# uclanlp/visualbert

Measured on NVIDIA H100. Metric: image-text pairs/sec fwd+bwd VisualBERT-base, higher is better.
Workload: dtype bf16

## Files before the change

include/vbert_b200.h:

```cpp
#ifndef VBERT_B200_H
#define VBERT_B200_H

#include <stdint.h>

#ifdef __cplusplus
extern "C" {
#endif

#define VB_ABI_VERSION 2

int vb_abi_version(void);
const char* vb_last_error(void);
int64_t vb_launch_count(void);
#define VB_PROFILE_CATEGORIES 11
void vb_profile_enable(int on);
int vb_profile_read(double* ms, double* work, int64_t* launches);

#define VB_EPI_NONE 0
#define VB_EPI_GELU 1
#define VB_EPI_DGELU 2

typedef struct {
    const void* A; int64_t lda; int32_t a_mn_major;
    const void* B; int64_t ldb; int32_t b_mn_major;
    int32_t M, N, K;
    void* D; int64_t ldd;
    int32_t d_fp32;
    int32_t splits;
    const float* bias;
    const void* addend; int64_t ld_add;
    int32_t epilogue;
    const void* aux_in;
    void* aux_out;
    int64_t ld_aux;
    float dropout_p; uint64_t dropout_seed; uint32_t dropout_stream;
    int32_t gp_tiled;
    const void* delta_ctx; float* delta_out; int32_t delta_seq;
} vb_gemm_args;
int vb_gemm_delta_ok(int32_t M, int32_t N);
int vb_gemm_gp_tiled_ok(int32_t M, int32_t N);

int vb_gemm(const vb_gemm_args* args, void* stream);

int vb_layernorm_fwd(const void* x, int64_t ldx, const float* gamma, const float* beta, void* y, int64_t ldy,
                     float* mean, float* rstd, int32_t rows, int32_t hidden, float eps, void* stream);
int vb_layernorm_bwd(const void* dy, const void* x, const float* mean, const float* rstd, const float* gamma,
                     void* dx, void* dx_drop, float* dgamma, float* dbeta, float* dbias, int32_t rows,
                     int32_t hidden, float dropout_p, uint64_t dropout_seed, uint32_t dropout_stream,
                     float in_dropout_p, uint32_t in_dropout_stream, void* stream);

int64_t vb_attention_keep_bytes(int32_t batch, int32_t seq, int32_t heads);
int vb_attention_fwd(const void* qkv, const float* mask_bias, void* ctx, float* lse, void* keep_mask, int32_t batch,
                     int32_t seq, int32_t heads, int32_t hidden, float dropout_p, uint64_t dropout_seed,
                     uint32_t dropout_stream, void* stream);
int vb_attention_bwd(const void* qkv, const float* mask_bias, const void* ctx, const float* lse, const void* keep_mask,
                     const void* dctx, void* dqkv, float* drow, int32_t batch, int32_t seq, int32_t heads,
                     int32_t hidden, float dropout_p, uint64_t dropout_seed, uint32_t dropout_stream, void* stream);

int vb_mask_bias(const int64_t* input_mask, const int64_t* image_mask, float* out, int32_t batch, int32_t text_len,
                 int32_t num_regions, void* stream);
int vb_cast_f32_to_bf16(const float* src, void* dst, int64_t n, void* stream);
int vb_cast_bf16_to_f32(const void* src, float* dst, int64_t n, void* stream);
#define VB_CAST_CHUNK 8192
typedef struct {
    const void* src;
    void* dst;
    int64_t numel;
    int32_t first_chunk;
    int32_t dst_fp32;
} vb_cast_item;
int vb_cast_multi(const vb_cast_item* table, int32_t n_items, int32_t n_chunks, void* stream);
int vb_colsum_bf16(const void* x, int64_t ld, float* out, int32_t rows, int32_t cols, void* stream);

int vb_cross_entropy_fwd(const void* logits, int64_t ld, const int64_t* labels, int32_t rows, int32_t vocab, float* lse,
                         float* loss_rows, void* stream);
int vb_cross_entropy_bwd(void* logits, int64_t ld, const int64_t* labels, int32_t rows, int32_t vocab, int32_t padded_cols,
                         const float* lse, const float* scale, void* stream);

typedef struct {
    int32_t batch, seq, hidden, heads, inter;
    float hidden_dropout, attn_dropout;
    uint64_t seed;
    uint32_t layer_index;
    const void* w_qkv;
    const void* w_attn_out;
    const void* w_inter;
    const void* w_out;
    const float* b_qkv;
    const float* b_attn_out; const float* ln1_gamma; const float* ln1_beta;
    const float* b_inter;
    const float* b_out; const float* ln2_gamma; const float* ln2_beta;
    const float* mask_bias;
} vb_layer_desc;

typedef struct {
    void* qkv;
    void* ctx;
    float* lse;
    void* pre1;
    float* mean1; float* rstd1;
    void* x1;
    void* u;
    void* g;
    void* pre2;
    float* mean2; float* rstd2;
    void* keep_mask;
} vb_layer_acts;

typedef struct {
    float* dw_qkv; float* db_qkv; float* dw_attn_out; float* db_attn_out; float* dln1_gamma; float* dln1_beta;
    float* dw_inter; float* db_inter; float* dw_out; float* db_out; float* dln2_gamma; float* dln2_beta;
} vb_layer_grads;

typedef struct {
    void* d_pre;
    void* d_pre_drop;
    void* d_big;
    void* d_x1;
    void* d_ctx;
    float* drow;
} vb_layer_scratch;

int vb_layer_fwd(const vb_layer_desc* d, const void* x_in, void* x_out, const vb_layer_acts* acts, void* stream);
int vb_layer_bwd(const vb_layer_desc* d, const void* x_in, const vb_layer_acts* acts, const void* dy, void* dx,
                 const vb_layer_grads* grads, const vb_layer_scratch* scratch, void* stream);

#define VB_ENCODER_ARENA_BUFFERS 14
int64_t vb_encoder_arena_layout(int32_t batch, int32_t seq, int32_t hidden, int32_t heads, int32_t inter, int32_t attn_dropout_on,
                                int64_t* offsets );
int vb_encoder_fwd(const vb_layer_desc* descs, int32_t n_layers, const void* x_in, void* arena, void* stream);
int vb_encoder_bwd(const vb_layer_desc* descs, int32_t n_layers, const void* x_in, void* arena, const void* dy, void* dx,
                   const vb_layer_grads* grads, const vb_layer_scratch* scratch, void* stream);

typedef struct {
    int32_t batch, text_len, num_regions, hidden, visual_dim, vocab, max_pos, n_types;
    float eps, dropout; uint64_t seed;
    const int64_t* input_ids;
    const int64_t* token_type_ids;
    const int64_t* visual_type;
    const void* visual_feats;
    const void* w_proj;
    const float* b_proj;
    const float* word; const float* pos; const float* type; const float* pos_vis; const float* type_vis;
    const float* gamma; const float* beta;
    const void* visual_addend;
} vb_embed_desc;

typedef struct {
    void* vis_proj;
    void* pre;
    float* mean; float* rstd;
} vb_embed_acts;

typedef struct {
    float* dword; float* dpos; float* dtype; float* dpos_vis; float* dtype_vis;
    float* dw_proj; float* db_proj; float* dgamma; float* dbeta;
    void* d_pre;
    void* d_vis;
    void* d_feats;
} vb_embed_grads;

int vb_embed_fwd(const vb_embed_desc* d, void* y, const vb_embed_acts* acts, void* stream);
int vb_embed_bwd(const vb_embed_desc* d, const vb_embed_acts* acts, const void* dy, const vb_embed_grads* g, void* stream);

#define VB_ADAM_CHUNK 32768
typedef struct {
    void* p;
    const void* g;
    void* m;
    void* v;
    int64_t numel;
    float lr;
    float weight_decay;
    int32_t first_chunk;
    int32_t reserved;
} vb_adam_tensor;
int vb_bert_adam_step(const vb_adam_tensor* table, int32_t n_tensors, int32_t n_chunks, float* sumsq, double b1, double b2,
                      double eps, double max_grad_norm, void* stream);

#ifdef __cplusplus
}
#endif
#endif
```

visualbert_b200/_lib.py:

```python
import ctypes
import os

_HERE = os.path.dirname(os.path.abspath(__file__))
LIB_PATH = os.environ.get("VB_LIB_PATH") or os.path.join(_HERE, "lib", "libvbert_b200.so")

ABI_VERSION = 2
VB_EPI_NONE, VB_EPI_GELU, VB_EPI_DGELU = 0, 1, 2

c_void_p, c_int, c_i64, c_f32, c_u64, c_u32 = (
    ctypes.c_void_p, ctypes.c_int32, ctypes.c_int64, ctypes.c_float, ctypes.c_uint64, ctypes.c_uint32)


class GemmArgs(ctypes.Structure):
    _fields_ = [
        ("A", c_void_p), ("lda", c_i64), ("a_mn_major", c_int),
        ("B", c_void_p), ("ldb", c_i64), ("b_mn_major", c_int),
        ("M", c_int), ("N", c_int), ("K", c_int),
        ("D", c_void_p), ("ldd", c_i64),
        ("d_fp32", c_int), ("splits", c_int),
        ("bias", c_void_p),
        ("addend", c_void_p), ("ld_add", c_i64),
        ("epilogue", c_int),
        ("aux_in", c_void_p), ("aux_out", c_void_p), ("ld_aux", c_i64),
        ("dropout_p", c_f32), ("dropout_seed", c_u64), ("dropout_stream", c_u32),
        ("gp_tiled", c_int),
        ("delta_ctx", c_void_p), ("delta_out", c_void_p), ("delta_seq", c_int),
    ]


def _struct(name, fields):
    return type(name, (ctypes.Structure,), {"_fields_": fields})


_P = c_void_p
LayerDesc = _struct("LayerDesc", [
    ("batch", c_int), ("seq", c_int), ("hidden", c_int), ("heads", c_int), ("inter", c_int),
    ("hidden_dropout", c_f32), ("attn_dropout", c_f32), ("seed", c_u64), ("layer_index", c_u32),
    ("w_qkv", _P), ("w_attn_out", _P), ("w_inter", _P), ("w_out", _P),
    ("b_qkv", _P), ("b_attn_out", _P), ("ln1_gamma", _P), ("ln1_beta", _P),
    ("b_inter", _P), ("b_out", _P), ("ln2_gamma", _P), ("ln2_beta", _P), ("mask_bias", _P)])
LayerActs = _struct("LayerActs", [(n, _P) for n in (
    "qkv", "ctx", "lse", "pre1", "mean1", "rstd1", "x1", "u", "g", "pre2", "mean2", "rstd2", "keep_mask")])
LayerGrads = _struct("LayerGrads", [(n, _P) for n in (
    "dw_qkv", "db_qkv", "dw_attn_out", "db_attn_out", "dln1_gamma", "dln1_beta",
    "dw_inter", "db_inter", "dw_out", "db_out", "dln2_gamma", "dln2_beta")])
LayerScratch = _struct("LayerScratch", [(n, _P) for n in ("d_pre", "d_pre_drop", "d_big", "d_x1", "d_ctx", "drow")])
EmbedDesc = _struct("EmbedDesc", [
    ("batch", c_int), ("text_len", c_int), ("num_regions", c_int), ("hidden", c_int), ("visual_dim", c_int),
    ("vocab", c_int), ("max_pos", c_int), ("n_types", c_int),
    ("eps", c_f32), ("dropout", c_f32), ("seed", c_u64),
    ("input_ids", _P), ("token_type_ids", _P), ("visual_type", _P), ("visual_feats", _P),
    ("w_proj", _P), ("b_proj", _P),
    ("word", _P), ("pos", _P), ("type", _P), ("pos_vis", _P), ("type_vis", _P), ("gamma", _P), ("beta", _P),
    ("visual_addend", _P)])
EmbedActs = _struct("EmbedActs", [(n, _P) for n in ("vis_proj", "pre", "mean", "rstd")])
EmbedGrads = _struct("EmbedGrads", [(n, _P) for n in (
    "dword", "dpos", "dtype", "dpos_vis", "dtype_vis", "dw_proj", "db_proj", "dgamma", "dbeta",
    "d_pre", "d_vis", "d_feats")])

AdamTensor = _struct("AdamTensor", [
    ("p", _P), ("g", _P), ("m", _P), ("v", _P), ("numel", c_i64), ("lr", c_f32), ("weight_decay", c_f32),
    ("first_chunk", c_int), ("reserved", c_int)])
VB_ADAM_CHUNK = 32768
CastItem = _struct("CastItem", [("src", _P), ("dst", _P), ("numel", c_i64), ("first_chunk", c_int), ("dst_fp32", c_int)])
VB_CAST_CHUNK = 8192

EXPORTS = [
    "vb_abi_version", "vb_last_error", "vb_launch_count", "vb_profile_enable", "vb_profile_read", "vb_gemm", "vb_gemm_gp_tiled_ok", "vb_gemm_delta_ok", "vb_layernorm_fwd", "vb_layernorm_bwd",
    "vb_attention_keep_bytes", "vb_attention_fwd", "vb_attention_bwd", "vb_mask_bias", "vb_cast_f32_to_bf16", "vb_cast_bf16_to_f32",
    "vb_colsum_bf16", "vb_cross_entropy_fwd", "vb_cross_entropy_bwd", "vb_layer_fwd", "vb_layer_bwd", "vb_embed_fwd", "vb_embed_bwd",
    "vb_bert_adam_step", "vb_cast_multi", "vb_encoder_arena_layout", "vb_encoder_fwd", "vb_encoder_bwd",
]
VB_ENCODER_ARENA_BUFFERS = 14
ARENA_NAMES = ("qkv", "ctx", "lse", "pre1", "mean1", "rstd1", "x1", "u", "g", "pre2", "mean2", "rstd2", "keep_mask", "y")


class VBertLibraryError(RuntimeError):
    pass


_lib = None


def lib():
    global _lib
    if _lib is None:
        if not os.path.exists(LIB_PATH):
            raise VBertLibraryError(
                f"{LIB_PATH} not found: build it with `python -c 'import __graft_entry__ as g; g.build()'`. "
                "visualbert_b200 has no CPU or PyTorch fallback.")
        h = ctypes.CDLL(LIB_PATH)
        h.vb_last_error.restype = ctypes.c_char_p
        h.vb_launch_count.restype = ctypes.c_int64
        h.vb_abi_version.restype = ctypes.c_int
        h.vb_attention_keep_bytes.restype = ctypes.c_int64
        h.vb_encoder_arena_layout.restype = ctypes.c_int64
        _lib = h
    return _lib


def check(rc, what):
    if rc != 0:
        msg = lib().vb_last_error().decode("utf-8", "replace")
        raise VBertLibraryError(f"{what} failed (status {rc}): {msg}")


def launch_count():
    return int(lib().vb_launch_count())


PROFILE_CATEGORIES = ("gemm_fwd", "gemm_dgrad", "gemm_wgrad", "attn_fwd", "attn_dq", "attn_dkv", "ln_fwd", "ln_bwd",
                      "colsum", "embed", "other")


def profile_enable(on=True):
    lib().vb_profile_enable(1 if on else 0)


def profile_read():
    k = len(PROFILE_CATEGORIES)
    ms = (ctypes.c_double * k)(); work = (ctypes.c_double * k)(); n = (ctypes.c_int64 * k)()
    check(lib().vb_profile_read(ms, work, n), "vb_profile_read")
    return {c: dict(ms=ms[i], work=work[i], launches=int(n[i])) for i, c in enumerate(PROFILE_CATEGORIES)}
```

visualbert_b200/csrc/vb_api.cu:

```cuda
#include <string.h>

#include "vb_internal.h"

namespace vb {

constexpr float kLnEps = 1e-12f;
constexpr unsigned kEmbedDropStream = 0xE0000001u;
enum { kSiteAttnProbs = 0, kSiteAttnOut = 1, kSiteFfnOut = 2 };
static inline unsigned drop_stream(unsigned layer, unsigned site) { return layer * 8u + site; }

#define VB_TRY(expr)            \
    do {                        \
        int _rc = (expr);       \
        if (_rc) return _rc;    \
    } while (0)

static vb_gemm_args fwd_args(const void* A, const void* W, void* D, int M, int N, int K) {
    vb_gemm_args a;
    memset(&a, 0, sizeof(a));
    a.A = A; a.lda = K; a.B = W; a.ldb = K; a.M = M; a.N = N; a.K = K; a.D = D; a.ldd = N;
    return a;
}
static vb_gemm_args dgrad_args(const void* dY, const void* W, void* dX, int M, int N, int K) {
    vb_gemm_args a;
    memset(&a, 0, sizeof(a));
    a.A = dY; a.lda = N; a.B = W; a.ldb = K; a.b_mn_major = 1; a.M = M; a.N = K; a.K = N; a.D = dX; a.ldd = K;
    return a;
}
static vb_gemm_args wgrad_args(const void* dY, const void* X, float* dW, int M, int N, int K) {
    vb_gemm_args a;
    memset(&a, 0, sizeof(a));
    a.A = dY; a.lda = N; a.a_mn_major = 1; a.B = X; a.ldb = K; a.b_mn_major = 1;
    a.M = N; a.N = K; a.K = M; a.D = dW; a.ldd = K; a.d_fp32 = 1;
    const int tiles = ((N + 127) / 128) * ((K + 255) / 256);
    int splits = (2 * num_sms()) / tiles;
    a.splits = splits < 1 ? 1 : splits;
    return a;
}

static int check_layer(const vb_layer_desc* d) {
    VB_REQUIRE(d != nullptr, "layer: null descriptor");
    VB_REQUIRE(d->batch > 0 && d->seq > 0, "layer: empty batch");
    VB_REQUIRE(d->hidden == d->heads * 64, "layer: hidden (%d) must equal heads (%d) * 64", d->hidden, d->heads);
    VB_REQUIRE(d->hidden % 16 == 0 && d->inter % 16 == 0, "layer: hidden/intermediate must be multiples of 16");
    VB_REQUIRE(d->w_qkv && d->w_attn_out && d->w_inter && d->w_out && d->mask_bias, "layer: null weight pointer");
    return 0;
}

int layer_fwd(const vb_layer_desc* d, const void* x_in, void* x_out, const vb_layer_acts* s, cudaStream_t st) {
    VB_TRY(check_layer(d));
    VB_REQUIRE(x_in && x_out && s, "layer_fwd: null pointer");
    const int M = d->batch * d->seq, H = d->hidden, I = d->inter;
    vb_gemm_args a = fwd_args(x_in, d->w_qkv, s->qkv, M, 3 * H, H);
    a.bias = d->b_qkv;
    static cudaEvent_t before_qkv[kMaxDevices] = {nullptr};
    const int dev = current_device();
    const bool want_mask = d->attn_dropout > 0.f && s->keep_mask != nullptr;
    if (want_mask) {
        if (before_qkv[dev] == nullptr) VB_CHECK_CUDA(cudaEventCreateWithFlags(&before_qkv[dev], cudaEventDisableTiming));
        VB_CHECK_CUDA(cudaEventRecord(before_qkv[dev], st));
    }
    VB_TRY(gemm(a, st));
    int mask_ready = 0;
    if (want_mask) {
        mask_ready = attn_mask_async(s->keep_mask, d->batch, d->seq, d->heads, H, d->attn_dropout, d->seed,
                                     drop_stream(d->layer_index, kSiteAttnProbs), before_qkv[dev], st);
        if (mask_ready < 0) return 2;
    }
    VB_TRY(attn_fwd(s->qkv, d->mask_bias, s->ctx, s->lse, s->keep_mask, d->batch, d->seq, d->heads, H, d->attn_dropout, d->seed,
                    drop_stream(d->layer_index, kSiteAttnProbs), st, mask_ready == 1));
    a = fwd_args(s->ctx, d->w_attn_out, s->pre1, M, H, H);
    a.bias = d->b_attn_out; a.addend = x_in; a.ld_add = H;
    a.dropout_p = d->hidden_dropout; a.dropout_seed = d->seed; a.dropout_stream = drop_stream(d->layer_index, kSiteAttnOut);
    VB_TRY(gemm(a, st));
    VB_TRY(ln_fwd(s->pre1, H, d->ln1_gamma, d->ln1_beta, s->x1, H, s->mean1, s->rstd1, M, H, kLnEps, st));
    a = fwd_args(s->x1, d->w_inter, s->u, M, I, H);
    a.bias = d->b_inter; a.epilogue = VB_EPI_GELU; a.aux_out = s->g; a.ld_aux = I;
    a.gp_tiled = gemm_gp_tiled_ok(M, I) ? 1 : 0;
    VB_TRY(gemm(a, st));
    a = fwd_args(s->g, d->w_out, s->pre2, M, H, I);
    a.bias = d->b_out; a.addend = s->x1; a.ld_add = H;
    a.dropout_p = d->hidden_dropout; a.dropout_seed = d->seed; a.dropout_stream = drop_stream(d->layer_index, kSiteFfnOut);
    VB_TRY(gemm(a, st));
    VB_TRY(ln_fwd(s->pre2, H, d->ln2_gamma, d->ln2_beta, x_out, H, s->mean2, s->rstd2, M, H, kLnEps, st));
    return 0;
}

int layer_bwd(const vb_layer_desc* d, const void* x_in, const vb_layer_acts* s, const void* dy, void* dx,
              const vb_layer_grads* g, const vb_layer_scratch* w, cudaStream_t st) {
    VB_TRY(check_layer(d));
    VB_REQUIRE(x_in && s && dy && dx && g && w, "layer_bwd: null pointer");
    const int M = d->batch * d->seq, H = d->hidden, I = d->inter;
    const bool hd = d->hidden_dropout > 0.f;
    VB_REQUIRE(!hd || w->d_pre_drop, "layer_bwd: d_pre_drop scratch required when hidden_dropout > 0");
    void* dpm = hd ? w->d_pre_drop : w->d_pre;

    VB_TRY(ln_bwd(dy, s->pre2, s->mean2, s->rstd2, d->ln2_gamma, w->d_pre, hd ? w->d_pre_drop : nullptr, g->dln2_gamma,
                  g->dln2_beta, g->db_out, M, H, d->hidden_dropout, d->seed, drop_stream(d->layer_index, kSiteFfnOut),
                  0.f, 0, st));
    VB_TRY(gemm(wgrad_args(dpm, s->g, g->dw_out, M, H, I), st));
    vb_gemm_args a = dgrad_args(dpm, d->w_out, w->d_big, M, H, I);
    a.epilogue = VB_EPI_DGELU; a.aux_in = s->u; a.ld_aux = I;
    a.gp_tiled = gemm_gp_tiled_ok(M, I) ? 1 : 0;
    VB_TRY(gemm(a, st));
    VB_TRY(colsum(w->d_big, I, g->db_inter, M, I, st));
    VB_TRY(gemm(wgrad_args(w->d_big, s->x1, g->dw_inter, M, I, H), st));
    a = dgrad_args(w->d_big, d->w_inter, w->d_x1, M, I, H);
    a.addend = w->d_pre; a.ld_add = H;
    VB_TRY(gemm(a, st));
    VB_TRY(ln_bwd(w->d_x1, s->pre1, s->mean1, s->rstd1, d->ln1_gamma, w->d_pre, hd ? w->d_pre_drop : nullptr,
                  g->dln1_gamma, g->dln1_beta, g->db_attn_out, M, H, d->hidden_dropout, d->seed,
                  drop_stream(d->layer_index, kSiteAttnOut), 0.f, 0, st));
    VB_TRY(gemm(wgrad_args(dpm, s->ctx, g->dw_attn_out, M, H, H), st));
    a = dgrad_args(dpm, d->w_attn_out, w->d_ctx, M, H, H);
    const bool fused_delta = gemm_delta_ok(M, H) && w->drow != nullptr &&
                             attn_bwd_takes_delta(s->qkv, w->d_ctx, w->d_big, d->batch, d->seq, d->heads, H);
    if (fused_delta) { a.delta_ctx = s->ctx; a.delta_out = w->drow; a.delta_seq = d->seq; }
    VB_TRY(gemm(a, st));
    VB_TRY(attn_bwd(s->qkv, d->mask_bias, s->ctx, s->lse, s->keep_mask, w->d_ctx, w->d_big, w->drow, d->batch, d->seq, d->heads, H,
                    d->attn_dropout, d->seed, drop_stream(d->layer_index, kSiteAttnProbs), st, fused_delta));
    VB_TRY(colsum(w->d_big, 3 * H, g->db_qkv, M, 3 * H, st));
    VB_TRY(gemm(wgrad_args(w->d_big, x_in, g->dw_qkv, M, 3 * H, H), st));
    a = dgrad_args(w->d_big, d->w_qkv, dx, M, 3 * H, H);
    a.addend = w->d_pre; a.ld_add = H;
    VB_TRY(gemm(a, st));
    return 0;
}

static long long align256(long long x) { return (x + 255) / 256 * 256; }

long long encoder_arena_layout(int B, int S, int H, int A, int I, int attn_drop, long long* off) {
    const long long M = static_cast<long long>(B) * S;
    const long long sizes[VB_ENCODER_ARENA_BUFFERS] = {
        M * 3 * H * 2, M * H * 2, static_cast<long long>(B) * A * S * 4, M * H * 2, M * 4, M * 4, M * H * 2, M * I * 2, M * I * 2,
        M * H * 2, M * 4, M * 4, attn_drop ? attn_keep_bytes(B, S, A) : 0, M * H * 2};
    long long o = 0;
    for (int i = 0; i < VB_ENCODER_ARENA_BUFFERS; ++i) {
        if (off) off[i] = o;
        o += align256(sizes[i]);
    }
    return o;
}

static void arena_acts(const vb_layer_desc* d, void* arena, int l, vb_layer_acts* a, void** y) {
    long long off[VB_ENCODER_ARENA_BUFFERS];
    const long long stride = encoder_arena_layout(d->batch, d->seq, d->hidden, d->heads, d->inter, d->attn_dropout > 0.f, off);
    char* base = static_cast<char*>(arena) + l * stride;
    a->qkv = base + off[0]; a->ctx = base + off[1]; a->lse = reinterpret_cast<float*>(base + off[2]);
    a->pre1 = base + off[3]; a->mean1 = reinterpret_cast<float*>(base + off[4]); a->rstd1 = reinterpret_cast<float*>(base + off[5]);
    a->x1 = base + off[6]; a->u = base + off[7]; a->g = base + off[8]; a->pre2 = base + off[9];
    a->mean2 = reinterpret_cast<float*>(base + off[10]); a->rstd2 = reinterpret_cast<float*>(base + off[11]);
    a->keep_mask = d->attn_dropout > 0.f ? base + off[12] : nullptr;
    *y = base + off[13];
}

int encoder_fwd(const vb_layer_desc* descs, int n, const void* x_in, void* arena, cudaStream_t st) {
    VB_REQUIRE(descs && n > 0 && x_in && arena, "encoder_fwd: null pointer / no layers");
    const void* x = x_in;
    for (int l = 0; l < n; ++l) {
        VB_REQUIRE(descs[l].batch == descs[0].batch && descs[l].seq == descs[0].seq && descs[l].hidden == descs[0].hidden &&
                   descs[l].heads == descs[0].heads && descs[l].inter == descs[0].inter &&
                   (descs[l].attn_dropout > 0.f) == (descs[0].attn_dropout > 0.f), "encoder_fwd: layers differ in shape");
        vb_layer_acts a;
        void* y;
        arena_acts(&descs[l], arena, l, &a, &y);
        VB_TRY(layer_fwd(&descs[l], x, y, &a, st));
        x = y;
    }
    return 0;
}

int encoder_bwd(const vb_layer_desc* descs, int n, const void* x_in, void* arena, const void* dy, void* dx,
                const vb_layer_grads* grads, const vb_layer_scratch* w, cudaStream_t st) {
    VB_REQUIRE(descs && n > 0 && x_in && arena && dy && dx && grads && w, "encoder_bwd: null pointer / no layers");
    const void* g_in = dy;
    for (int l = n - 1; l >= 0; --l) {
        vb_layer_acts a;
        void* y;
        arena_acts(&descs[l], arena, l, &a, &y);
        const void* xl = x_in;
        if (l > 0) {
            vb_layer_acts ap;
            void* yp;
            arena_acts(&descs[l - 1], arena, l - 1, &ap, &yp);
            xl = yp;
        }
        VB_TRY(layer_bwd(&descs[l], xl, &a, g_in, dx, &grads[l], w, st));
        g_in = dx;
    }
    return 0;
}

static int check_embed(const vb_embed_desc* d) {
    VB_REQUIRE(d != nullptr, "embed: null descriptor");
    VB_REQUIRE(d->batch > 0 && d->text_len > 0 && d->num_regions >= 0, "embed: bad shape");
    VB_REQUIRE(d->hidden % 16 == 0, "embed: hidden must be a multiple of 16");
    VB_REQUIRE(d->num_regions == 0 || (d->visual_dim % 8 == 0 && d->visual_feats && d->w_proj && d->visual_type),
               "embed: visual inputs missing or visual_dim not a multiple of 8");
    return 0;
}

int embed_fwd_api(const vb_embed_desc* d, void* y, const vb_embed_acts* s, cudaStream_t st) {
    VB_TRY(check_embed(d));
    VB_REQUIRE(y && s && s->pre && s->mean && s->rstd, "embed_fwd: null pointer");
    const int BV = d->batch * d->num_regions;
    if (BV > 0) {
        vb_gemm_args a = fwd_args(d->visual_feats, d->w_proj, s->vis_proj, BV, d->hidden, d->visual_dim);
        a.bias = d->b_proj;
        if (d->visual_addend != nullptr) {
            a.addend = d->visual_addend;
            a.ld_add = d->hidden;
        }
        VB_TRY(gemm(a, st));
    }
    EmbedParams p;
    memset(&p, 0, sizeof(p));
    p.ids = reinterpret_cast<const long long*>(d->input_ids);
    p.tt = reinterpret_cast<const long long*>(d->token_type_ids);
    p.vt = reinterpret_cast<const long long*>(d->visual_type);
    p.vis_proj = static_cast<const bf16*>(s->vis_proj);
    p.word = d->word; p.pos = d->pos; p.type = d->type; p.pos_vis = d->pos_vis; p.type_vis = d->type_vis;
    p.gamma = d->gamma; p.beta = d->beta;
    p.pre = static_cast<bf16*>(s->pre); p.y = static_cast<bf16*>(y); p.mean = s->mean; p.rstd = s->rstd;
    p.B = d->batch; p.T = d->text_len; p.V = d->num_regions; p.H = d->hidden;
    p.vocab = d->vocab; p.max_pos = d->max_pos; p.n_types = d->n_types;
    p.eps = d->eps;
    if (d->dropout > 0.f) {
        const DropQ q = dropout_quantise(d->dropout);
        p.drop_scale = q.scale;
        p.drop_thresh16 = q.thr8;
        p.drop_seed = d->seed;
        p.drop_stream = kEmbedDropStream;
    }
    return embed_fwd(p, st);
}

int embed_bwd_api(const vb_embed_desc* d, const vb_embed_acts* s, const void* dy, const vb_embed_grads* g,
                  cudaStream_t st) {
    VB_TRY(check_embed(d));
    VB_REQUIRE(s && dy && g && g->d_pre, "embed_bwd: null pointer");
    const int M = d->batch * (d->text_len + d->num_regions), H = d->hidden, BV = d->batch * d->num_regions;
    VB_TRY(ln_bwd(dy, s->pre, s->mean, s->rstd, d->gamma, g->d_pre, nullptr, g->dgamma, g->dbeta, nullptr, M, H, 0.f,
                  d->seed, 0, d->dropout, kEmbedDropStream, st));
    EmbedBwdParams p;
    memset(&p, 0, sizeof(p));
    p.de = static_cast<const bf16*>(g->d_pre);
    p.ids = reinterpret_cast<const long long*>(d->input_ids);
    p.tt = reinterpret_cast<const long long*>(d->token_type_ids);
    p.vt = reinterpret_cast<const long long*>(d->visual_type);
    p.dword = g->dword; p.dpos = g->dpos; p.dtype = g->dtype; p.dpos_vis = g->dpos_vis; p.dtype_vis = g->dtype_vis;
    p.dvis = static_cast<bf16*>(g->d_vis);
    p.B = d->batch; p.T = d->text_len; p.V = d->num_regions; p.H = H;
    p.vocab = d->vocab; p.max_pos = d->max_pos; p.n_types = d->n_types;
    VB_TRY(embed_bwd(p, st));
    if (BV > 0) {
        VB_TRY(colsum(g->d_vis, H, g->db_proj, BV, H, st));
        VB_TRY(gemm(wgrad_args(g->d_vis, d->visual_feats, g->dw_proj, BV, H, d->visual_dim), st));
        if (g->d_feats) VB_TRY(gemm(dgrad_args(g->d_vis, d->w_proj, g->d_feats, BV, H, d->visual_dim), st));
    }
    return 0;
}

}

extern "C" {
int vb_layer_fwd(const vb_layer_desc* d, const void* x_in, void* x_out, const vb_layer_acts* acts, void* stream) {
    return vb::layer_fwd(d, x_in, x_out, acts, static_cast<cudaStream_t>(stream));
}
int vb_layer_bwd(const vb_layer_desc* d, const void* x_in, const vb_layer_acts* acts, const void* dy, void* dx,
                 const vb_layer_grads* grads, const vb_layer_scratch* scratch, void* stream) {
    return vb::layer_bwd(d, x_in, acts, dy, dx, grads, scratch, static_cast<cudaStream_t>(stream));
}
int64_t vb_encoder_arena_layout(int32_t batch, int32_t seq, int32_t hidden, int32_t heads, int32_t inter, int32_t attn_dropout_on,
                                int64_t* offsets) {
    long long off[VB_ENCODER_ARENA_BUFFERS];
    const long long stride = vb::encoder_arena_layout(batch, seq, hidden, heads, inter, attn_dropout_on, off);
    if (offsets) for (int i = 0; i < VB_ENCODER_ARENA_BUFFERS; ++i) offsets[i] = off[i];
    return stride;
}
int vb_encoder_fwd(const vb_layer_desc* descs, int32_t n_layers, const void* x_in, void* arena, void* stream) {
    return vb::encoder_fwd(descs, n_layers, x_in, arena, static_cast<cudaStream_t>(stream));
}
int vb_encoder_bwd(const vb_layer_desc* descs, int32_t n_layers, const void* x_in, void* arena, const void* dy, void* dx,
                   const vb_layer_grads* grads, const vb_layer_scratch* scratch, void* stream) {
    return vb::encoder_bwd(descs, n_layers, x_in, arena, dy, dx, grads, scratch, static_cast<cudaStream_t>(stream));
}
int vb_embed_fwd(const vb_embed_desc* d, void* y, const vb_embed_acts* acts, void* stream) {
    return vb::embed_fwd_api(d, y, acts, static_cast<cudaStream_t>(stream));
}
int vb_embed_bwd(const vb_embed_desc* d, const vb_embed_acts* acts, const void* dy, const vb_embed_grads* g, void* stream) {
    return vb::embed_bwd_api(d, acts, dy, g, static_cast<cudaStream_t>(stream));
}
int vb_mask_bias(const int64_t* input_mask, const int64_t* image_mask, float* out, int32_t batch, int32_t text_len,
                 int32_t num_regions, void* stream) {
    return vb::mask_bias(reinterpret_cast<const long long*>(input_mask), reinterpret_cast<const long long*>(image_mask),
                         out, batch, text_len, num_regions, static_cast<cudaStream_t>(stream));
}
int vb_cast_f32_to_bf16(const float* src, void* dst, int64_t n, void* stream) {
    return vb::cast_f32_bf16(src, dst, n, static_cast<cudaStream_t>(stream));
}
int vb_cast_bf16_to_f32(const void* src, float* dst, int64_t n, void* stream) {
    return vb::cast_bf16_f32(src, dst, n, static_cast<cudaStream_t>(stream));
}
int vb_colsum_bf16(const void* x, int64_t ld, float* out, int32_t rows, int32_t cols, void* stream) {
    return vb::colsum(x, ld, out, rows, cols, static_cast<cudaStream_t>(stream));
}
}
```

visualbert_b200/csrc/vb_common.cuh:

```cuda
#pragma once

#include <cuda.h>
#include <cuda_bf16.h>
#include <cuda_runtime.h>
#include <stdint.h>
#include <stdio.h>

#include <atomic>

namespace vb {

typedef __nv_bfloat16 bf16;

extern std::atomic<long long> g_launches;
int num_sms();
constexpr int kMaxDevices = 64;
int current_device();
template <typename K>
inline cudaError_t ensure_dyn_smem(K kern, int bytes, int (&cache)[kMaxDevices]) {
    const int d = current_device();
    if (cache[d] >= bytes) return cudaSuccess;
    cudaError_t e = cudaFuncSetAttribute(kern, cudaFuncAttributeMaxDynamicSharedMemorySize, bytes);
    if (e == cudaSuccess) cache[d] = bytes;
    return e;
}

enum { PROF_GEMM_FWD = 0, PROF_GEMM_DGRAD = 1, PROF_GEMM_WGRAD = 2, PROF_ATTN_FWD = 3, PROF_ATTN_DQ = 4, PROF_ATTN_DKV = 5,
       PROF_LN_FWD = 6, PROF_LN_BWD = 7, PROF_COLSUM = 8, PROF_EMBED = 9, PROF_OTHER = 10, PROF_NCAT = 11 };
bool pdl_enabled();
#ifdef __CUDACC__
__device__ __forceinline__ void pdl_wait() { asm volatile("griddepcontrol.wait;" ::: "memory"); }
__device__ __forceinline__ void pdl_trigger() { asm volatile("griddepcontrol.launch_dependents;" ::: "memory"); }
template <typename... KArgs, typename... Args>
inline cudaError_t launch_pdl(void (*kernel)(KArgs...), dim3 grid, dim3 block, size_t smem, cudaStream_t st, Args&&... args) {
    cudaLaunchConfig_t cfg = {};
    cfg.gridDim = grid;
    cfg.blockDim = block;
    cfg.dynamicSmemBytes = smem;
    cfg.stream = st;
    cudaLaunchAttribute attr[1];
    attr[0].id = cudaLaunchAttributeProgrammaticStreamSerialization;
    attr[0].val.programmaticStreamSerializationAllowed = 1;
    cfg.attrs = attr;
    cfg.numAttrs = pdl_enabled() ? 1 : 0;
    return cudaLaunchKernelEx(&cfg, kernel, static_cast<KArgs>(args)...);
}
#endif

struct ProfScope {
    ProfScope(cudaStream_t st, int cat, double work, int launches);
    ~ProfScope();
    int slot;
    cudaStream_t st;
};

void set_error(const char* fmt, ...);
#define VB_CHECK_CUDA(expr)                                                                   \
    do {                                                                                      \
        cudaError_t _e = (expr);                                                              \
        if (_e != cudaSuccess) {                                                              \
            vb::set_error("%s:%d: %s -> %s", __FILE__, __LINE__, #expr, cudaGetErrorString(_e)); \
            return 1;                                                                         \
        }                                                                                     \
    } while (0)
#define VB_REQUIRE(cond, ...)                                                                 \
    do {                                                                                      \
        if (!(cond)) {                                                                        \
            vb::set_error(__VA_ARGS__);                                                       \
            return 2;                                                                         \
        }                                                                                     \
    } while (0)

__device__ __forceinline__ uint32_t smem_u32(const void* p) {
    return static_cast<uint32_t>(__cvta_generic_to_shared(p));
}

__device__ __forceinline__ float warp_sum(float v) {
#pragma unroll
    for (int o = 16; o > 0; o >>= 1) v += __shfl_xor_sync(0xffffffffu, v, o);
    return v;
}
__device__ __forceinline__ float warp_max(float v) {
#pragma unroll
    for (int o = 16; o > 0; o >>= 1) v = fmaxf(v, __shfl_xor_sync(0xffffffffu, v, o));
    return v;
}

__device__ __forceinline__ uint32_t pack_bf16x2(float lo, float hi) {
    __nv_bfloat162 h = __floats2bfloat162_rn(lo, hi);
    return *reinterpret_cast<uint32_t*>(&h);
}
__device__ __forceinline__ float2 unpack_bf16x2(uint32_t v) {
    __nv_bfloat162 h = *reinterpret_cast<__nv_bfloat162*>(&v);
    return __bfloat1622float2(h);
}

__device__ __forceinline__ float fast_ex2(float x) {
    float r;
    asm("ex2.approx.ftz.f32 %0, %1;" : "=f"(r) : "f"(x));
    return r;
}
__device__ __forceinline__ float fast_rcp(float x) {
    float r;
    asm("rcp.approx.ftz.f32 %0, %1;" : "=f"(r) : "f"(x));
    return r;
}

__device__ __forceinline__ float erfc_abs_sqrt2(float x, float& e) {
    const float ax = fabsf(x);
    e = fast_ex2(x * x * -0.72134752044448170f);
    const float t = fast_rcp(fmaf(0.23164189f, ax, 1.0f));
    float poly = fmaf(1.061405429f, t, -1.453152027f);
    poly = fmaf(poly, t, 1.421413741f);
    poly = fmaf(poly, t, -0.284496736f);
    poly = fmaf(poly, t, 0.254829592f);
    return poly * t * e;
}
__device__ __forceinline__ float gelu_fwd(float x) {
    float e;
    const float q = erfc_abs_sqrt2(x, e);
    const float hx = 0.5f * x, ha = fabsf(hx);
    return fmaf(-ha, q, hx + ha);
}
__device__ __forceinline__ void gelu_fwd_bwd(float x, float& g, float& gp) {
    float e;
    const float q = erfc_abs_sqrt2(x, e);
    const float cdf = 0.5f + copysignf(fmaf(-0.5f, q, 0.5f), x);
    g = x * cdf;
    gp = fmaf(x * e, 0.3989422804014327f, cdf);
}
__device__ __forceinline__ float gelu_bwd(float x) {
    float e;
    const float q = erfc_abs_sqrt2(x, e);
    const float cdf = 0.5f + copysignf(fmaf(-0.5f, q, 0.5f), x);
    return fmaf(x * e, 0.3989422804014327f, cdf);
}

__device__ __forceinline__ uint32_t mix32(uint32_t x) {
    x ^= x >> 16; x *= 0x7feb352du;
    x ^= x >> 15; x *= 0x846ca68bu;
    x ^= x >> 16;
    return x;
}
__device__ __forceinline__ uint32_t dropout_key(uint64_t seed, uint32_t stream) {
    return mix32(static_cast<uint32_t>(seed) ^ mix32(static_cast<uint32_t>(seed >> 32) + 0x9E3779B9u * (stream + 1u)));
}
struct DropQ { unsigned thr8; float scale; };
inline DropQ dropout_quantise(float p) {
    DropQ q;
    unsigned n = static_cast<unsigned>(p * 256.0f + 0.5f);
    if (n > 255u) n = 255u;
    q.thr8 = n;
    q.scale = p > 0.f ? 256.0f / (256.0f - static_cast<float>(n)) : 0.f;
    return q;
}
__device__ __forceinline__ uint32_t dropout_keep8(uint64_t seed, uint32_t stream, uint64_t elem8, uint32_t thr8) {
    const uint32_t key = dropout_key(seed, stream) ^ (static_cast<uint32_t>(elem8 >> 31) * 0x27d4eb2fu);
    const uint32_t base = static_cast<uint32_t>(elem8) << 1;
    const uint32_t t4 = thr8 * 0x01010101u;
    const uint32_t m0 = __vcmpgeu4(mix32(base ^ key), t4) & 0x01010101u;
    const uint32_t m1 = __vcmpgeu4(mix32((base + 1u) ^ key), t4) & 0x01010101u;
    return ((m0 * 0x01020408u) >> 24) | (((m1 * 0x01020408u) >> 24) << 4);
}

__device__ __forceinline__ void mbar_init(uint32_t bar, uint32_t count) {
    asm volatile("mbarrier.init.shared::cta.b64 [%0], %1;" ::"r"(bar), "r"(count) : "memory");
}
__device__ __forceinline__ void fence_barrier_init() {
    asm volatile("fence.mbarrier_init.release.cluster;" ::: "memory");
}
__device__ __forceinline__ void fence_proxy_async_smem() {
    asm volatile("fence.proxy.async.shared::cta;" ::: "memory");
}
__device__ __forceinline__ void mbar_arrive(uint32_t bar) {
    asm volatile("mbarrier.arrive.shared::cta.b64 _, [%0];" ::"r"(bar) : "memory");
}
__device__ __forceinline__ void mbar_arrive_expect_tx(uint32_t bar, uint32_t bytes) {
    asm volatile("mbarrier.arrive.expect_tx.shared::cta.b64 _, [%0], %1;" ::"r"(bar), "r"(bytes)
                 : "memory");
}
__device__ __forceinline__ bool mbar_try_wait(uint32_t bar, uint32_t parity) {
    uint32_t ok;
    asm volatile(
        "{\n"
        ".reg .pred p;\n"
        "mbarrier.try_wait.parity.shared::cta.b64 p, [%1], %2;\n"
        "selp.u32 %0, 1, 0, p;\n"
        "}\n"
        : "=r"(ok)
        : "r"(bar), "r"(parity)
        : "memory");
    return ok != 0;
}
__device__ __forceinline__ void mbar_wait(uint32_t bar, uint32_t parity) {
    if (mbar_try_wait(bar, parity)) return;
    const long long t0 = clock64();
    uint32_t spins = 0;
    while (!mbar_try_wait(bar, parity)) {
        if ((++spins & 0x3ffu) == 0 && clock64() - t0 > 4000000000ll) __trap();
    }
}

__device__ __forceinline__ void tma_prefetch_desc(const CUtensorMap* m) {
    asm volatile("prefetch.tensormap [%0];" ::"l"(reinterpret_cast<uint64_t>(m)) : "memory");
}
__device__ __forceinline__ void tma_load_2d(uint32_t smem_dst, const CUtensorMap* m, uint32_t bar,
                                            int c_inner, int c_outer) {
    asm volatile(
        "cp.async.bulk.tensor.2d.shared::cluster.global.mbarrier::complete_tx::bytes"
        " [%0], [%1, {%3, %4}], [%2];"
        ::"r"(smem_dst), "l"(reinterpret_cast<uint64_t>(m)), "r"(bar), "r"(c_inner), "r"(c_outer)
        : "memory");
}

__device__ __forceinline__ uint64_t wgmma_desc_sw128(uint32_t saddr, uint32_t lbo_bytes, uint32_t sbo_bytes) {
    return static_cast<uint64_t>((saddr & 0x3FFFFu) >> 4) | (static_cast<uint64_t>((lbo_bytes >> 4) & 0x3FFFu) << 16) |
           (static_cast<uint64_t>((sbo_bytes >> 4) & 0x3FFFu) << 32) | (1ull << 62);
}
__device__ __forceinline__ void wgmma_fence() { asm volatile("wgmma.fence.sync.aligned;" ::: "memory"); }
__device__ __forceinline__ void wgmma_commit() { asm volatile("wgmma.commit_group.sync.aligned;" ::: "memory"); }
template <int N>
__device__ __forceinline__ void wgmma_wait() { asm volatile("wgmma.wait_group.sync.aligned %0;" ::"n"(N) : "memory"); }
template <int TA, int TB>
__device__ __forceinline__ void wgmma_m64n128k16(float (&d)[64], uint64_t a_desc, uint64_t b_desc, uint32_t accumulate) {
    asm volatile(
        "{\n"
        ".reg .pred p;\n"
        "setp.ne.b32 p, %66, 0;\n"
        "wgmma.mma_async.sync.aligned.m64n128k16.f32.bf16.bf16 "
        "{%0, %1, %2, %3, %4, %5, %6, %7, %8, %9, %10, %11, %12, %13, %14, %15, %16, %17, %18, %19, %20, %21, %22, %23, %24, %25, %26, %27, %28, %29, %30, %31, %32, %33, %34, %35, %36, %37, %38, %39, %40, %41, %42, %43, %44, %45, %46, %47, %48, %49, %50, %51, %52, %53, %54, %55, %56, %57, %58, %59, %60, %61, %62, %63}, "
        "%64, %65, p, 1, 1, %67, %68;\n"
        "}\n"
        : "+f"(d[0]), "+f"(d[1]), "+f"(d[2]), "+f"(d[3]), "+f"(d[4]), "+f"(d[5]), "+f"(d[6]), "+f"(d[7]),
          "+f"(d[8]), "+f"(d[9]), "+f"(d[10]), "+f"(d[11]), "+f"(d[12]), "+f"(d[13]), "+f"(d[14]), "+f"(d[15]),
          "+f"(d[16]), "+f"(d[17]), "+f"(d[18]), "+f"(d[19]), "+f"(d[20]), "+f"(d[21]), "+f"(d[22]), "+f"(d[23]),
          "+f"(d[24]), "+f"(d[25]), "+f"(d[26]), "+f"(d[27]), "+f"(d[28]), "+f"(d[29]), "+f"(d[30]), "+f"(d[31]),
          "+f"(d[32]), "+f"(d[33]), "+f"(d[34]), "+f"(d[35]), "+f"(d[36]), "+f"(d[37]), "+f"(d[38]), "+f"(d[39]),
          "+f"(d[40]), "+f"(d[41]), "+f"(d[42]), "+f"(d[43]), "+f"(d[44]), "+f"(d[45]), "+f"(d[46]), "+f"(d[47]),
          "+f"(d[48]), "+f"(d[49]), "+f"(d[50]), "+f"(d[51]), "+f"(d[52]), "+f"(d[53]), "+f"(d[54]), "+f"(d[55]),
          "+f"(d[56]), "+f"(d[57]), "+f"(d[58]), "+f"(d[59]), "+f"(d[60]), "+f"(d[61]), "+f"(d[62]), "+f"(d[63])
        : "l"(a_desc), "l"(b_desc), "r"(accumulate), "n"(TA), "n"(TB));
}
template <int TA, int TB>
__device__ __forceinline__ void wgmma_m64n64k16_ss(float (&d)[32], uint64_t a_desc, uint64_t b_desc, uint32_t accumulate) {
    asm volatile(
        "{\n"
        ".reg .pred p;\n"
        "setp.ne.b32 p, %34, 0;\n"
        "wgmma.mma_async.sync.aligned.m64n64k16.f32.bf16.bf16 "
        "{%0, %1, %2, %3, %4, %5, %6, %7, %8, %9, %10, %11, %12, %13, %14, %15, %16, %17, %18, %19, %20, %21, %22, %23, %24, %25, %26, %27, %28, %29, %30, %31}, "
        "%32, %33, p, 1, 1, %35, %36;\n"
        "}\n"
        : "+f"(d[0]), "+f"(d[1]), "+f"(d[2]), "+f"(d[3]), "+f"(d[4]), "+f"(d[5]), "+f"(d[6]), "+f"(d[7]),
          "+f"(d[8]), "+f"(d[9]), "+f"(d[10]), "+f"(d[11]), "+f"(d[12]), "+f"(d[13]), "+f"(d[14]), "+f"(d[15]),
          "+f"(d[16]), "+f"(d[17]), "+f"(d[18]), "+f"(d[19]), "+f"(d[20]), "+f"(d[21]), "+f"(d[22]), "+f"(d[23]),
          "+f"(d[24]), "+f"(d[25]), "+f"(d[26]), "+f"(d[27]), "+f"(d[28]), "+f"(d[29]), "+f"(d[30]), "+f"(d[31])
        : "l"(a_desc), "l"(b_desc), "r"(accumulate), "n"(TA), "n"(TB));
}
template <int TB>
__device__ __forceinline__ void wgmma_m64n64k16_rs(float (&d)[32], const uint32_t (&a)[4], uint64_t b_desc, uint32_t accumulate) {
    asm volatile(
        "{\n"
        ".reg .pred p;\n"
        "setp.ne.b32 p, %37, 0;\n"
        "wgmma.mma_async.sync.aligned.m64n64k16.f32.bf16.bf16 "
        "{%0, %1, %2, %3, %4, %5, %6, %7, %8, %9, %10, %11, %12, %13, %14, %15, %16, %17, %18, %19, %20, %21, %22, %23, %24, %25, %26, %27, %28, %29, %30, %31}, "
        "{%32, %33, %34, %35}, %36, p, 1, 1, %38;\n"
        "}\n"
        : "+f"(d[0]), "+f"(d[1]), "+f"(d[2]), "+f"(d[3]), "+f"(d[4]), "+f"(d[5]), "+f"(d[6]), "+f"(d[7]),
          "+f"(d[8]), "+f"(d[9]), "+f"(d[10]), "+f"(d[11]), "+f"(d[12]), "+f"(d[13]), "+f"(d[14]), "+f"(d[15]),
          "+f"(d[16]), "+f"(d[17]), "+f"(d[18]), "+f"(d[19]), "+f"(d[20]), "+f"(d[21]), "+f"(d[22]), "+f"(d[23]),
          "+f"(d[24]), "+f"(d[25]), "+f"(d[26]), "+f"(d[27]), "+f"(d[28]), "+f"(d[29]), "+f"(d[30]), "+f"(d[31])
        : "r"(a[0]), "r"(a[1]), "r"(a[2]), "r"(a[3]), "l"(b_desc), "r"(accumulate), "n"(TB));
}
__device__ __forceinline__ bool elect_one() {
    uint32_t pred;
    asm volatile(
        "{\n"
        ".reg .pred P1;\n"
        "elect.sync _|P1, 0xffffffff;\n"
        "selp.u32 %0, 1, 0, P1;\n"
        "}\n"
        : "=r"(pred));
    return pred != 0;
}
template <int N>
__device__ __forceinline__ void reg_dec() { asm volatile("setmaxnreg.dec.sync.aligned.u32 %0;" ::"n"(N)); }
template <int N>
__device__ __forceinline__ void reg_inc() { asm volatile("setmaxnreg.inc.sync.aligned.u32 %0;" ::"n"(N)); }
__device__ __forceinline__ void named_bar_sync(int id, int nthreads) {
    asm volatile("bar.sync %0, %1;" ::"r"(id), "r"(nthreads) : "memory");
}

__device__ __forceinline__ uint4 ldg_v4(const void* p) {
    return __ldg(reinterpret_cast<const uint4*>(p));
}
__device__ __forceinline__ void stg_v4(void* p, uint4 v) { *reinterpret_cast<uint4*>(p) = v; }
__device__ __forceinline__ void ldg_v8(const void* p, uint32_t (&r)[8]) {
    const uint4 a = ldg_v4(p), b = ldg_v4(static_cast<const uint8_t*>(p) + 16);
    r[0] = a.x; r[1] = a.y; r[2] = a.z; r[3] = a.w; r[4] = b.x; r[5] = b.y; r[6] = b.z; r[7] = b.w;
}
__device__ __forceinline__ void stg_v8(void* p, const uint32_t (&r)[8]) {
    stg_v4(p, make_uint4(r[0], r[1], r[2], r[3]));
    stg_v4(static_cast<uint8_t*>(p) + 16, make_uint4(r[4], r[5], r[6], r[7]));
}
__device__ __forceinline__ void red_add_v4_f32(float* p, float a, float b, float c, float d) {
    asm volatile("red.global.add.v4.f32 [%0], {%1, %2, %3, %4};" ::"l"(p), "f"(a), "f"(b), "f"(c),
                 "f"(d)
                 : "memory");
}

}
```

visualbert_b200/csrc/vb_gemm.cu:

```cuda
#include <stdarg.h>
#include <stdio.h>
#include <stdlib.h>
#include <string.h>

#include <atomic>
#include <mutex>
#include <vector>

#include "../../include/vbert_b200.h"
#include "vb_common.cuh"

namespace vb {

static thread_local char g_err[1024] = "";
std::atomic<long long> g_launches{0};

void set_error(const char* fmt, ...) {
    va_list ap;
    va_start(ap, fmt);
    vsnprintf(g_err, sizeof(g_err), fmt, ap);
    va_end(ap);
}
const char* get_error() { return g_err; }

struct ProfRec { cudaEvent_t e0, e1; int cat; double work; int launches; };
static bool g_prof_on = false;
static std::vector<ProfRec> g_prof;
static std::vector<ProfRec> g_prof_pool;
static std::mutex g_prof_mu;

ProfScope::ProfScope(cudaStream_t s, int cat, double work, int launches) : slot(-1), st(s) {
    g_launches.fetch_add(launches);
    if (!g_prof_on) return;
    std::lock_guard<std::mutex> lk(g_prof_mu);
    ProfRec r;
    if (!g_prof_pool.empty()) { r = g_prof_pool.back(); g_prof_pool.pop_back(); }
    else { cudaEventCreate(&r.e0); cudaEventCreate(&r.e1); }
    r.cat = cat; r.work = work; r.launches = launches;
    cudaEventRecord(r.e0, st);
    g_prof.push_back(r);
    slot = static_cast<int>(g_prof.size()) - 1;
}
ProfScope::~ProfScope() {
    if (slot < 0) return;
    std::lock_guard<std::mutex> lk(g_prof_mu);
    cudaEventRecord(g_prof[slot].e1, st);
}

constexpr int BLOCK_M = 128;
constexpr int BLOCK_K = 64;
constexpr int WGMMA_K = 16;
constexpr int kStages = 4;
constexpr int kEpiWarps = 8;
constexpr int kThreads = 128 + kEpiWarps * 32;
constexpr int kAtomBytes = 64 * BLOCK_K * 2;

template <int BLOCK_N>
struct Cfg {
    static constexpr int A_BYTES = BLOCK_M * BLOCK_K * 2;
    static constexpr int B_BYTES = BLOCK_N * BLOCK_K * 2;
    static constexpr int STAGE_BYTES = A_BYTES + B_BYTES;
    static constexpr int ACC_LD = BLOCK_N + 4;
    static constexpr int RING_BYTES = kStages * STAGE_BYTES > BLOCK_M * ACC_LD * 4 ? kStages * STAGE_BYTES : BLOCK_M * ACC_LD * 4;
    static constexpr int BAR_OFF = RING_BYTES;
    static constexpr int NUM_BARS = 2 * kStages;
    static constexpr int BIAS_OFF = BAR_OFF + NUM_BARS * 8;
    static constexpr int SMEM_BYTES = BIAS_OFF + BLOCK_N * 4 + 1024;
    static_assert(SMEM_BYTES <= 227 * 1024, "shared memory per block");
};

struct GemmParams {
    int M, N, K;
    int splits;
    void* D; long long ldd;
    const float* bias;
    const bf16* addend; long long ld_add;
    int epilogue;
    const bf16* aux_in;
    bf16* aux_out; long long ld_aux;
    float drop_scale;
    unsigned drop_thresh16;
    unsigned long long drop_seed;
    unsigned drop_stream;
    int m_fast;
    float* delta_out;
    int delta_seq;
};
bool gemm_gp_tiled_ok(int M, int N);
bool gemm_delta_ok(int M, int N);

struct TileCoord {
    int m_blk, n_blk, kb_begin, kb_end;
};
__device__ __forceinline__ TileCoord decode_tile(int t, int n_blocks, int splits, int k_blocks, int m_blocks, bool m_fast) {
    TileCoord c;
    const int split = t % splits;
    const int mn = t / splits;
    if (m_fast) {
        c.m_blk = mn % m_blocks;
        c.n_blk = mn / m_blocks;
    } else {
        c.n_blk = mn % n_blocks;
        c.m_blk = mn / n_blocks;
    }
    c.kb_begin = static_cast<int>(static_cast<long long>(split) * k_blocks / splits);
    c.kb_end = static_cast<int>(static_cast<long long>(split + 1) * k_blocks / splits);
    return c;
}

__device__ __forceinline__ void load16_bf16(const bf16* p, float (&f)[16]) {
    uint32_t r[8];
    ldg_v8(p, r);
#pragma unroll
    for (int i = 0; i < 8; ++i) {
        const float2 t = unpack_bf16x2(r[i]);
        f[2 * i] = t.x;
        f[2 * i + 1] = t.y;
    }
}
__device__ __forceinline__ void store16_bf16(bf16* p, const float (&f)[16]) {
    uint32_t r[8];
#pragma unroll
    for (int i = 0; i < 8; ++i) r[i] = pack_bf16x2(f[2 * i], f[2 * i + 1]);
    stg_v8(p, r);
}

enum { EPI_GENERIC = 0, EPI_BIAS = 1, EPI_RESID = 2, EPI_DROP_RESID = 3, EPI_GELU_FWD = 4, EPI_DGELU_BWD = 5, EPI_GELU_FWD_T = 6,
       EPI_DGELU_BWD_T = 7, EPI_DELTA = 8 };
__host__ __device__ constexpr bool epi_is_gelu(int e) { return e == EPI_GELU_FWD || e == EPI_GELU_FWD_T; }
__host__ __device__ constexpr bool epi_is_dgelu(int e) { return e == EPI_DGELU_BWD || e == EPI_DGELU_BWD_T; }

template <bool OUT_F32, int EPI = EPI_GENERIC, bool TO_REGS = false>
__device__ __forceinline__ void epilogue16(const GemmParams& p, int row, int col, const float* sbias, const uint32_t (&ex)[8],
                                           float (&x)[16], uint32_t* o0 = nullptr, uint32_t* o1 = nullptr) {
    if (sbias != nullptr) {
#pragma unroll
        for (int i = 0; i < 4; ++i) {
            const float4 b = *reinterpret_cast<const float4*>(sbias + 4 * i);
            x[4 * i] += b.x; x[4 * i + 1] += b.y; x[4 * i + 2] += b.z; x[4 * i + 3] += b.w;
        }
    }
    if constexpr (OUT_F32) {
        float* d = reinterpret_cast<float*>(p.D) + static_cast<long long>(row) * p.ldd + col;
#pragma unroll
        for (int i = 0; i < 4; ++i) red_add_v4_f32(d + 4 * i, x[4 * i], x[4 * i + 1], x[4 * i + 2], x[4 * i + 3]);
    } else {
        constexpr bool kGeneric = EPI == EPI_GENERIC;
        if (EPI == EPI_DROP_RESID || (kGeneric && p.drop_scale != 0.0f)) {
            const unsigned long long e8 =
                (static_cast<unsigned long long>(row) * static_cast<unsigned>(p.N) + col) >> 3;
#pragma unroll
            for (int h = 0; h < 2; ++h) {
                const uint32_t keep = dropout_keep8(p.drop_seed, p.drop_stream, e8 + h, p.drop_thresh16);
#pragma unroll
                for (int i = 0; i < 8; ++i) x[8 * h + i] = ((keep >> i) & 1u) ? x[8 * h + i] * p.drop_scale : 0.0f;
            }
        }
        if (EPI == EPI_RESID || EPI == EPI_DROP_RESID || (kGeneric && p.addend != nullptr)) {
#pragma unroll
            for (int i = 0; i < 8; ++i) {
                const float2 t = unpack_bf16x2(ex[i]);
                x[2 * i] += t.x;
                x[2 * i + 1] += t.y;
            }
        }
        bf16* d = reinterpret_cast<bf16*>(p.D) + static_cast<long long>(row) * p.ldd + col;
        if (epi_is_gelu(EPI) || (kGeneric && p.epilogue == VB_EPI_GELU)) {
            float gp[16];
#pragma unroll
            for (int i = 0; i < 16; ++i) gelu_fwd_bwd(x[i], x[i], gp[i]);
            if constexpr (TO_REGS) {
#pragma unroll
                for (int i = 0; i < 8; ++i) { o0[i] = pack_bf16x2(gp[2 * i], gp[2 * i + 1]); o1[i] = pack_bf16x2(x[2 * i], x[2 * i + 1]); }
                return;
            }
            store16_bf16(d, gp);
            d = p.aux_out + static_cast<long long>(row) * p.ld_aux + col;
        } else if (kGeneric && p.epilogue == 3) {
            store16_bf16(d, x);
            d = p.aux_out + static_cast<long long>(row) * p.ld_aux + col;
        } else if (epi_is_dgelu(EPI) || (kGeneric && p.epilogue == VB_EPI_DGELU)) {
#pragma unroll
            for (int i = 0; i < 8; ++i) {
                const float2 t = unpack_bf16x2(ex[i]);
                x[2 * i] *= t.x;
                x[2 * i + 1] *= t.y;
            }
        }
        if constexpr (TO_REGS) {
#pragma unroll
            for (int i = 0; i < 8; ++i) o0[i] = pack_bf16x2(x[2 * i], x[2 * i + 1]);
            return;
        }
        store16_bf16(d, x);
    }
}

template <bool A_MN, bool B_MN, int BLOCK_N, bool OUT_F32, int EPI = EPI_GENERIC>
__global__ void __launch_bounds__(kThreads, 1)
gemm_wgmma_kernel(const __grid_constant__ CUtensorMap tmA, const __grid_constant__ CUtensorMap tmB, const GemmParams p) {
    using C = Cfg<BLOCK_N>;
    static_assert(BLOCK_N % 128 == 0, "64 x 128 wgmma pieces");
    static_assert(!(EPI == EPI_GELU_FWD_T || EPI == EPI_DGELU_BWD_T) || BLOCK_N == 256, "tile-native gelu' is defined on 256-wide tiles");
    extern __shared__ uint8_t smem_raw[];
    const uint32_t raw = smem_u32(smem_raw);
    const uint32_t base = (raw + 1023u) & ~1023u;
    uint8_t* smem = smem_raw + (base - raw);

    const int warp = threadIdx.x >> 5;
    const int lane = threadIdx.x & 31;

    auto a_tile = [&](int s) { return base + s * C::STAGE_BYTES; };
    auto b_tile = [&](int s) { return base + s * C::STAGE_BYTES + C::A_BYTES; };
    auto full_bar = [&](int s) { return base + C::BAR_OFF + 8 * s; };
    auto empty_bar = [&](int s) { return base + C::BAR_OFF + 8 * (kStages + s); };

    if (threadIdx.x == 0) {
        tma_prefetch_desc(&tmA);
        tma_prefetch_desc(&tmB);
        for (int s = 0; s < kStages; ++s) {
            mbar_init(full_bar(s), 1);
            mbar_init(empty_bar(s), 2);
        }
        fence_barrier_init();
    }
    __syncthreads();
    pdl_trigger();
    pdl_wait();

    const int m_blocks = (p.M + BLOCK_M - 1) / BLOCK_M;
    const int n_blocks = (p.N + BLOCK_N - 1) / BLOCK_N;
    const int k_blocks = (p.K + BLOCK_K - 1) / BLOCK_K;
    const TileCoord tc = decode_tile(blockIdx.x, n_blocks, p.splits, k_blocks, m_blocks, p.m_fast != 0);

    if (warp < 4) {
        reg_dec<40>();
        if (warp == 0) {
            int stage = 0;
            uint32_t phase = 0;
            for (int kb = tc.kb_begin; kb < tc.kb_end; ++kb) {
                mbar_wait(empty_bar(stage), phase ^ 1u);
                if (elect_one()) {
                    mbar_arrive_expect_tx(full_bar(stage), C::STAGE_BYTES);
                    if constexpr (!A_MN) {
                        tma_load_2d(a_tile(stage), &tmA, full_bar(stage), kb * BLOCK_K, tc.m_blk * BLOCK_M);
                    } else {
#pragma unroll
                        for (int i = 0; i < BLOCK_M / 64; ++i)
                            tma_load_2d(a_tile(stage) + i * kAtomBytes, &tmA, full_bar(stage), tc.m_blk * BLOCK_M + i * 64, kb * BLOCK_K);
                    }
                    if constexpr (!B_MN) {
                        tma_load_2d(b_tile(stage), &tmB, full_bar(stage), kb * BLOCK_K, tc.n_blk * BLOCK_N);
                    } else {
#pragma unroll
                        for (int i = 0; i < BLOCK_N / 64; ++i)
                            tma_load_2d(b_tile(stage) + i * kAtomBytes, &tmB, full_bar(stage), tc.n_blk * BLOCK_N + i * 64, kb * BLOCK_K);
                    }
                }
                __syncwarp();
                if (++stage == kStages) { stage = 0; phase ^= 1u; }
            }
        }
        return;
    }
    reg_inc<232>();

    const int wg = (warp >> 2) - 1;
    const int et = threadIdx.x - 128;
    float* sbias = reinterpret_cast<float*>(smem + C::BIAS_OFF);
    const bool has_bias = p.bias != nullptr;
    if (has_bias) {
        const bool mine = p.splits == 1 || (blockIdx.x % p.splits) == 0;
        for (int i = et; i < BLOCK_N; i += kEpiWarps * 32) {
            const int col = tc.n_blk * BLOCK_N + i;
            sbias[i] = (mine && col < p.N) ? __ldg(p.bias + col) : 0.f;
        }
    }
    constexpr int NH = BLOCK_N / 128;
    constexpr uint32_t a_kstep = A_MN ? WGMMA_K * 128 : WGMMA_K * 2;
    constexpr uint32_t b_kstep = B_MN ? WGMMA_K * 128 : WGMMA_K * 2;
    float acc[NH][64];
    {
        int stage = 0, prev = 0;
        uint32_t phase = 0;
        for (int kb = tc.kb_begin; kb < tc.kb_end; ++kb) {
            mbar_wait(full_bar(stage), phase);
            const uint32_t a0 = a_tile(stage) + wg * 8192, b0 = b_tile(stage);
            wgmma_fence();
#pragma unroll
            for (int k = 0; k < BLOCK_K / WGMMA_K; ++k) {
                const uint64_t ad = wgmma_desc_sw128(a0 + k * a_kstep, kAtomBytes, 1024);
#pragma unroll
                for (int h = 0; h < NH; ++h)
                    wgmma_m64n128k16<A_MN ? 1 : 0, B_MN ? 1 : 0>(acc[h], ad, wgmma_desc_sw128(b0 + h * 16384 + k * b_kstep, kAtomBytes, 1024),
                                                                 (kb > tc.kb_begin || k > 0) ? 1u : 0u);
            }
            wgmma_commit();
            wgmma_wait<1>();
            if (kb > tc.kb_begin && (threadIdx.x & 127) == 0) mbar_arrive(empty_bar(prev));
            prev = stage;
            if (++stage == kStages) { stage = 0; phase ^= 1u; }
        }
        wgmma_wait<0>();
    }

    const int ew = warp - 4;
    const int q = ew & 3, half = ew >> 2;
    const int lrow = q * 32 + lane;
    const int row = tc.m_blk * BLOCK_M + lrow;
    const int col0 = tc.n_blk * BLOCK_N + half * (BLOCK_N / 2);
    constexpr int NCH = BLOCK_N / 2 / 16;
    const long long gp_tile_off =
        ((((static_cast<long long>(tc.m_blk >> 1) * n_blocks + tc.n_blk) * 2 + (tc.m_blk & 1)) * kEpiWarps + ew) * NCH) * 512 + lane * 16;
    const bf16* exb = nullptr;
    long long ex_step = 16;
    if constexpr (!OUT_F32) {
        constexpr bool kWantAdd = EPI == EPI_RESID || EPI == EPI_DROP_RESID || EPI == EPI_DELTA;
        if (row < p.M) {
            if (kWantAdd || (EPI == EPI_GENERIC && p.addend != nullptr)) exb = p.addend + static_cast<long long>(row) * p.ld_add + col0;
            else if (EPI == EPI_DGELU_BWD || (EPI == EPI_GENERIC && p.epilogue == VB_EPI_DGELU))
                exb = p.aux_in + static_cast<long long>(row) * p.ld_aux + col0;
            else if (EPI == EPI_DGELU_BWD_T) { exb = p.aux_in + gp_tile_off; ex_step = 512; }
        }
    }
    constexpr bool kEx = !OUT_F32 && EPI != EPI_BIAS && !epi_is_gelu(EPI);
    uint32_t ex[kEx ? NCH : 1][8];
    if constexpr (kEx) {
#pragma unroll
        for (int k = 0; k < NCH; ++k)
            if (exb != nullptr && col0 + k * 16 < p.N) ldg_v8(exb + k * ex_step, ex[k]);
    }

    named_bar_sync(1, kEpiWarps * 32);
    float* sacc = reinterpret_cast<float*>(smem);
    {
        const int r0 = wg * 64 + ((warp & 3) << 4) + (lane >> 2);
#pragma unroll
        for (int h = 0; h < NH; ++h)
#pragma unroll
            for (int j = 0; j < 16; ++j)
#pragma unroll
                for (int i = 0; i < 2; ++i)
                    *reinterpret_cast<float2*>(sacc + (r0 + 8 * i) * C::ACC_LD + h * 128 + j * 8 + 2 * (lane & 3)) =
                        make_float2(acc[h][4 * j + 2 * i], acc[h][4 * j + 2 * i + 1]);
    }
    named_bar_sync(1, kEpiWarps * 32);

    const float* srow = sacc + lrow * C::ACC_LD + half * (BLOCK_N / 2);
    [[maybe_unused]] float hsum = 0.f;
#pragma unroll
    for (int k = 0; k < NCH; ++k) {
        const int col = col0 + k * 16;
        if (row < p.M && col < p.N) {
            float x[16];
#pragma unroll
            for (int i = 0; i < 4; ++i) {
                const float4 v = *reinterpret_cast<const float4*>(srow + k * 16 + 4 * i);
                x[4 * i] = v.x; x[4 * i + 1] = v.y; x[4 * i + 2] = v.z; x[4 * i + 3] = v.w;
            }
            const float* sb = has_bias ? sbias + half * (BLOCK_N / 2) + k * 16 : nullptr;
            const uint32_t (&e)[8] = ex[kEx ? k : 0];
            if constexpr (EPI == EPI_GELU_FWD_T) {
                uint32_t o0[8], o1[8];
                epilogue16<OUT_F32, EPI, true>(p, row, col, sb, e, x, o0, o1);
                stg_v8(reinterpret_cast<bf16*>(p.D) + gp_tile_off + k * 512, o0);
                stg_v8(p.aux_out + static_cast<long long>(row) * p.ld_aux + col, o1);
            } else if constexpr (EPI == EPI_DELTA) {
                uint32_t o0[8];
                epilogue16<OUT_F32, EPI, true>(p, row, col, sb, e, x, o0);
                stg_v8(reinterpret_cast<bf16*>(p.D) + static_cast<long long>(row) * p.ldd + col, o0);
#pragma unroll
                for (int i = 0; i < 8; ++i) {
                    const float2 a = unpack_bf16x2(o0[i]), b = unpack_bf16x2(e[i]);
                    hsum = fmaf(a.x, b.x, fmaf(a.y, b.y, hsum));
                }
            } else {
                epilogue16<OUT_F32, EPI>(p, row, col, sb, e, x);
            }
        }
        if constexpr (EPI == EPI_DELTA) {
            if ((k & 3) == 3) {
                const int c4 = col - 48;
                if (row < p.M && c4 < p.N) {
                    const int bi = row / p.delta_seq, si = row - bi * p.delta_seq;
                    p.delta_out[(static_cast<long long>(bi) * (p.N >> 6) + (c4 >> 6)) * p.delta_seq + si] = hsum;
                }
                hsum = 0.f;
            }
        }
    }
}

typedef CUresult (*EncodeTiledFn)(CUtensorMap*, CUtensorMapDataType, cuuint32_t, void*, const cuuint64_t*,
                                  const cuuint64_t*, const cuuint32_t*, const cuuint32_t*,
                                  CUtensorMapInterleave, CUtensorMapSwizzle, CUtensorMapL2promotion,
                                  CUtensorMapFloatOOBfill);

static EncodeTiledFn get_encode_fn() {
    static EncodeTiledFn fn = nullptr;
    static bool tried = false;
    if (!tried) {
        tried = true;
        void* sym = nullptr;
        cudaDriverEntryPointQueryResult qres;
        if (cudaGetDriverEntryPoint("cuTensorMapEncodeTiled", &sym, cudaEnableDefault, &qres) == cudaSuccess &&
            qres == cudaDriverEntryPointSuccess)
            fn = reinterpret_cast<EncodeTiledFn>(sym);
    }
    return fn;
}

struct TmapKey {
    const void* ptr; uint64_t d0, d1, d2, s0, s1; uint32_t b0, b1, b2, rank; int dev;
    bool operator==(const TmapKey& o) const {
        return ptr == o.ptr && d0 == o.d0 && d1 == o.d1 && d2 == o.d2 && s0 == o.s0 && s1 == o.s1 && b0 == o.b0 && b1 == o.b1 && b2 == o.b2 &&
               rank == o.rank && dev == o.dev;
    }
};
struct TmapSlot { TmapKey key; CUtensorMap map; bool used; };
constexpr int kTmapSlots = 4096;
static thread_local std::vector<TmapSlot>* g_tmap_cache = nullptr;

static int encode_tmap_cached(CUtensorMap* m, const void* ptr, uint32_t rank, const cuuint64_t* dims, const cuuint64_t* strides,
                              const cuuint32_t* box) {
    TmapKey k;
    memset(&k, 0, sizeof(k));
    k.ptr = ptr; k.rank = rank; k.dev = current_device();
    k.d0 = dims[0]; k.d1 = dims[1]; k.d2 = rank > 2 ? dims[2] : 1;
    k.s0 = strides[0]; k.s1 = rank > 2 ? strides[1] : 0;
    k.b0 = box[0]; k.b1 = box[1]; k.b2 = rank > 2 ? box[2] : 1;
    uint64_t h = reinterpret_cast<uintptr_t>(ptr) * 0x9E3779B97F4A7C15ull;
    h ^= (k.d0 * 31 + k.d1) * 0xBF58476D1CE4E5B9ull + k.d2 * 1315423911ull + k.s0 * 2654435761ull + k.s1 * 40503ull;
    h ^= (static_cast<uint64_t>(k.b1) << 20) ^ (static_cast<uint64_t>(k.b0) << 8) ^ k.b2 ^ (static_cast<uint64_t>(k.dev) << 40);
    h ^= h >> 29;
    if (g_tmap_cache == nullptr) { g_tmap_cache = new std::vector<TmapSlot>(kTmapSlots); for (auto& sl : *g_tmap_cache) sl.used = false; }
    TmapSlot& sl = (*g_tmap_cache)[h & (kTmapSlots - 1)];
    if (sl.used && sl.key == k) { *m = sl.map; return 0; }
    EncodeTiledFn fn = get_encode_fn();
    VB_REQUIRE(fn != nullptr, "cuTensorMapEncodeTiled unavailable (driver too old / no GPU?)");
    cuuint32_t estr[3] = {1, 1, 1};
    CUresult r = fn(m, CU_TENSOR_MAP_DATA_TYPE_BFLOAT16, rank, const_cast<void*>(ptr), dims, strides, box, estr,
                    CU_TENSOR_MAP_INTERLEAVE_NONE, CU_TENSOR_MAP_SWIZZLE_128B, CU_TENSOR_MAP_L2_PROMOTION_L2_256B,
                    CU_TENSOR_MAP_FLOAT_OOB_FILL_NONE);
    VB_REQUIRE(r == CUDA_SUCCESS, "cuTensorMapEncodeTiled (rank %u) failed with CUresult %d", rank, static_cast<int>(r));
    sl.key = k; sl.map = *m; sl.used = true;
    return 0;
}

int make_tmap_bf16(CUtensorMap* m, const void* ptr, uint64_t inner, uint64_t outer, uint64_t ld_elems,
                   uint32_t box_outer) {
    VB_REQUIRE((reinterpret_cast<uintptr_t>(ptr) & 15) == 0, "TMA operand not 16-byte aligned");
    VB_REQUIRE((ld_elems * 2) % 16 == 0, "TMA operand row stride must be a multiple of 8 elements");
    cuuint64_t dims[2] = {inner, outer};
    cuuint64_t strides[1] = {ld_elems * 2};
    cuuint32_t box[2] = {64, box_outer};
    return encode_tmap_cached(m, ptr, 2, dims, strides, box);
}

int current_device() {
    int dev = 0;
    cudaGetDevice(&dev);
    return (dev < 0 || dev >= kMaxDevices) ? 0 : dev;
}

int num_sms() {
    static int n[kMaxDevices] = {0};
    const int dev = current_device();
    if (n[dev] == 0) {
        int v = 0;
        cudaDeviceGetAttribute(&v, cudaDevAttrMultiProcessorCount, dev);
        n[dev] = v > 0 ? v : 132;
    }
    return n[dev];
}

template <bool A_MN, bool B_MN, int BLOCK_N, bool OUT_F32, int EPI = EPI_GENERIC>
static int launch(const CUtensorMap& ta, const CUtensorMap& tb, const GemmParams& p, cudaStream_t st) {
    using C = Cfg<BLOCK_N>;
    auto kern = gemm_wgmma_kernel<A_MN, B_MN, BLOCK_N, OUT_F32, EPI>;
    static int configured[kMaxDevices] = {0};
    VB_CHECK_CUDA(ensure_dyn_smem(kern, C::SMEM_BYTES, configured));
    const long long tiles = static_cast<long long>((p.M + BLOCK_M - 1) / BLOCK_M) * ((p.N + BLOCK_N - 1) / BLOCK_N) * p.splits;
    VB_REQUIRE(tiles < (1LL << 31), "vb_gemm: too many tiles");
    {
        ProfScope ps(st, OUT_F32 ? PROF_GEMM_WGRAD : (B_MN ? PROF_GEMM_DGRAD : PROF_GEMM_FWD), 2.0 * p.M * p.N * p.K, 1);
        VB_CHECK_CUDA(launch_pdl(kern, dim3(static_cast<unsigned>(tiles)), dim3(kThreads), C::SMEM_BYTES, st, ta, tb, p));
    }
    VB_CHECK_CUDA(cudaGetLastError());
    return 0;
}

bool pdl_enabled() {
    static const bool on = [] {
        const char* e = getenv("VB_PDL");
        return !(e && e[0] == '0');
    }();
    return on;
}

bool gemm_delta_ok(int M, int N) {
    static const int off = [] { const char* e = getenv("VB_GEMM_DELTA"); return (e != nullptr && atoi(e) == 0) ? 1 : 0; }();
    const int n_pad256 = (N + 255) / 256 * 256;
    return !off && M >= 256 && N >= 256 && N % 64 == 0 && (n_pad256 - N) * 8 <= N;
}
bool gemm_gp_tiled_ok(int M, int N) {
    static const int off = [] { const char* e = getenv("VB_GEMM_GP_TILED"); return (e != nullptr && atoi(e) == 0) ? 1 : 0; }();
    return !off && M >= 256 && M % 256 == 0 && N % 256 == 0;
}

int gemm(const vb_gemm_args& a, cudaStream_t st) {
    VB_REQUIRE(a.M > 0 && a.N > 0 && a.K > 0, "vb_gemm: empty problem M=%d N=%d K=%d", a.M, a.N, a.K);
    VB_REQUIRE(a.N % 16 == 0, "vb_gemm: N=%d must be a multiple of 16", a.N);
    VB_REQUIRE(a.A && a.B && a.D, "vb_gemm: null operand");
    VB_REQUIRE(a.ldd % 16 == 0 && (reinterpret_cast<uintptr_t>(a.D) & 31) == 0, "vb_gemm: D must be 32-byte aligned with ldd a multiple of 16");
    VB_REQUIRE(!a.addend || (a.ld_add % 16 == 0 && (reinterpret_cast<uintptr_t>(a.addend) & 31) == 0), "vb_gemm: addend must be 32-byte aligned with ld a multiple of 16");
    VB_REQUIRE((!a.aux_in && !a.aux_out) || a.ld_aux % 16 == 0, "vb_gemm: ld_aux must be a multiple of 16");
    VB_REQUIRE((reinterpret_cast<uintptr_t>(a.aux_in) & 31) == 0 && (reinterpret_cast<uintptr_t>(a.aux_out) & 31) == 0,
               "vb_gemm: aux_in / aux_out must be 32-byte aligned");
    VB_REQUIRE(a.epilogue == VB_EPI_NONE || a.epilogue == VB_EPI_GELU || a.epilogue == VB_EPI_DGELU || a.epilogue == 3,
               "vb_gemm: unknown epilogue %d", a.epilogue);
    VB_REQUIRE(a.epilogue != VB_EPI_GELU || a.aux_out, "vb_gemm: GELU epilogue needs aux_out");
    VB_REQUIRE(a.epilogue != VB_EPI_DGELU || a.aux_in, "vb_gemm: DGELU epilogue needs aux_in");
    VB_REQUIRE(!a.d_fp32 || (a.epilogue == VB_EPI_NONE && !a.addend && a.dropout_p == 0.0f),
               "vb_gemm: fp32-accumulate output supports bias only");
    VB_REQUIRE(a.dropout_p >= 0.0f && a.dropout_p < 1.0f, "vb_gemm: dropout_p out of range");
    VB_REQUIRE(!a.delta_out || (gemm_delta_ok(a.M, a.N) && a.delta_ctx && a.delta_seq > 0 && a.M % a.delta_seq == 0 && !a.d_fp32 &&
                                !a.a_mn_major && a.b_mn_major && !a.bias && !a.addend && a.dropout_p == 0.0f && a.epilogue == VB_EPI_NONE &&
                                (reinterpret_cast<uintptr_t>(a.delta_ctx) & 31) == 0),
               "vb_gemm: delta_out needs a plain bf16 input-gradient GEMM (b_mn_major, no bias / addend / dropout) and vb_gemm_delta_ok(M, N)");
    VB_REQUIRE(!a.gp_tiled || (gemm_gp_tiled_ok(a.M, a.N) && !a.d_fp32 && !a.a_mn_major && (a.epilogue == VB_EPI_GELU || a.epilogue == VB_EPI_DGELU)),
               "vb_gemm: gp_tiled needs a GELU / DGELU epilogue and vb_gemm_gp_tiled_ok(M, N)");
    VB_REQUIRE(!a.gp_tiled || a.epilogue != VB_EPI_DGELU || a.b_mn_major,
               "vb_gemm: gp_tiled with the DGELU epilogue needs an MN-major B (the input-gradient GEMM)");
    VB_REQUIRE(!a.gp_tiled || a.epilogue != VB_EPI_GELU || !a.b_mn_major, "vb_gemm: gp_tiled with the GELU epilogue needs a K-major B");

    GemmParams p;
    memset(&p, 0, sizeof(p));
    p.M = a.M; p.N = a.N; p.K = a.K;
    const int k_blocks = (a.K + BLOCK_K - 1) / BLOCK_K;
    int splits = (a.d_fp32 && a.splits > 1) ? a.splits : 1;
    if (splits > k_blocks) splits = k_blocks;
    p.splits = splits;
    p.D = a.D; p.ldd = a.ldd;
    p.bias = a.bias;
    p.addend = static_cast<const bf16*>(a.addend); p.ld_add = a.ld_add;
    p.epilogue = a.epilogue;
    p.aux_in = static_cast<const bf16*>(a.aux_in);
    p.aux_out = static_cast<bf16*>(a.aux_out);
    p.ld_aux = a.ld_aux;
    if (a.delta_out) {
        p.addend = static_cast<const bf16*>(a.delta_ctx); p.ld_add = a.N;
        p.delta_out = a.delta_out; p.delta_seq = a.delta_seq;
    }
    {
        static const int order_off = [] { const char* e = getenv("VB_GEMM_TILE_ORDER"); return (e != nullptr && atoi(e) == 0) ? 1 : 0; }();
        p.m_fast = (!order_off && (a.M + BLOCK_M - 1) / BLOCK_M < (a.N + 255) / 256) ? 1 : 0;
    }
    if (a.dropout_p > 0.0f) {
        const DropQ q = dropout_quantise(a.dropout_p);
        p.drop_scale = q.scale;
        p.drop_thresh16 = q.thr8;
        p.drop_seed = a.dropout_seed;
        p.drop_stream = a.dropout_stream;
    }

    const int n_pad256 = (a.N + 255) / 256 * 256;
    const bool bn256 = (a.N >= 256) && ((n_pad256 - a.N) * 8 <= a.N);
    VB_REQUIRE(!a.delta_out || bn256, "vb_gemm: delta_out needs 256-wide tiles");

    CUtensorMap ta, tb;
    int rc;
    if (!a.a_mn_major) rc = make_tmap_bf16(&ta, a.A, a.K, a.M, a.lda, BLOCK_M);
    else               rc = make_tmap_bf16(&ta, a.A, a.M, a.K, a.lda, BLOCK_K);
    if (rc) return rc;
    if (!a.b_mn_major) rc = make_tmap_bf16(&tb, a.B, a.K, a.N, a.ldb, bn256 ? 256 : 128);
    else               rc = make_tmap_bf16(&tb, a.B, a.N, a.K, a.ldb, BLOCK_K);
    if (rc) return rc;

    if (bn256 && !a.d_fp32) {
        const bool drop = a.dropout_p > 0.0f, add = a.addend != nullptr;
        int epi = EPI_GENERIC;
        if (a.epilogue == VB_EPI_GELU && !drop && !add) epi = a.gp_tiled ? EPI_GELU_FWD_T : EPI_GELU_FWD;
        else if (a.epilogue == VB_EPI_DGELU && !drop && !add) epi = a.gp_tiled ? EPI_DGELU_BWD_T : EPI_DGELU_BWD;
        else if (a.epilogue == VB_EPI_NONE) epi = add ? (drop ? EPI_DROP_RESID : EPI_RESID) : (drop ? EPI_GENERIC : EPI_BIAS);
        if (a.delta_out) epi = EPI_DELTA;
        VB_REQUIRE(!a.gp_tiled || epi == EPI_GELU_FWD_T || epi == EPI_DGELU_BWD_T,
                   "vb_gemm: gp_tiled needs a plain GELU / DGELU epilogue (no dropout, no addend)");
        if (!a.a_mn_major && !a.b_mn_major) {
            switch (epi) {
                case EPI_BIAS: return launch<false, false, 256, false, EPI_BIAS>(ta, tb, p, st);
                case EPI_RESID: return launch<false, false, 256, false, EPI_RESID>(ta, tb, p, st);
                case EPI_DROP_RESID: return launch<false, false, 256, false, EPI_DROP_RESID>(ta, tb, p, st);
                case EPI_GELU_FWD: return launch<false, false, 256, false, EPI_GELU_FWD>(ta, tb, p, st);
                case EPI_GELU_FWD_T: return launch<false, false, 256, false, EPI_GELU_FWD_T>(ta, tb, p, st);
                default: return launch<false, false, 256, false>(ta, tb, p, st);
            }
        }
        if (!a.a_mn_major && a.b_mn_major) {
            switch (epi) {
                case EPI_BIAS: return launch<false, true, 256, false, EPI_BIAS>(ta, tb, p, st);
                case EPI_RESID: return launch<false, true, 256, false, EPI_RESID>(ta, tb, p, st);
                case EPI_DGELU_BWD: return launch<false, true, 256, false, EPI_DGELU_BWD>(ta, tb, p, st);
                case EPI_DELTA: return launch<false, true, 256, false, EPI_DELTA>(ta, tb, p, st);
                case EPI_DGELU_BWD_T: return launch<false, true, 256, false, EPI_DGELU_BWD_T>(ta, tb, p, st);
                default: return launch<false, true, 256, false>(ta, tb, p, st);
            }
        }
    }

#define VB_DISPATCH(AM, BM, F32)                                         \
    (bn256 ? launch<AM, BM, 256, F32>(ta, tb, p, st) : launch<AM, BM, 128, F32>(ta, tb, p, st))
    if (!a.d_fp32) {
        if (!a.a_mn_major && !a.b_mn_major) return VB_DISPATCH(false, false, false);
        if (!a.a_mn_major && a.b_mn_major) return VB_DISPATCH(false, true, false);
        if (a.a_mn_major && a.b_mn_major) return VB_DISPATCH(true, true, false);
        return VB_DISPATCH(true, false, false);
    } else {
        if (!a.a_mn_major && !a.b_mn_major) return VB_DISPATCH(false, false, true);
        if (!a.a_mn_major && a.b_mn_major) return VB_DISPATCH(false, true, true);
        if (a.a_mn_major && a.b_mn_major) return VB_DISPATCH(true, true, true);
        return VB_DISPATCH(true, false, true);
    }
#undef VB_DISPATCH
}

}

extern "C" {
int vb_abi_version(void) { return VB_ABI_VERSION; }
const char* vb_last_error(void) { return vb::get_error(); }
int64_t vb_launch_count(void) { return vb::g_launches.load(); }
void vb_profile_enable(int on) {
    std::lock_guard<std::mutex> lk(vb::g_prof_mu);
    vb::g_prof_on = on != 0;
}
int vb_profile_read(double* ms, double* work, int64_t* launches) {
    if (cudaDeviceSynchronize() != cudaSuccess) { vb::set_error("vb_profile_read: device sync failed"); return 1; }
    std::lock_guard<std::mutex> lk(vb::g_prof_mu);
    for (int c = 0; c < vb::PROF_NCAT; ++c) { ms[c] = 0; work[c] = 0; launches[c] = 0; }
    for (auto& r : vb::g_prof) {
        float t = 0.f;
        cudaEventElapsedTime(&t, r.e0, r.e1);
        ms[r.cat] += t; work[r.cat] += r.work; launches[r.cat] += r.launches;
        vb::g_prof_pool.push_back(r);
    }
    vb::g_prof.clear();
    return 0;
}
int vb_gemm_delta_ok(int32_t M, int32_t N) { return vb::gemm_delta_ok(M, N) ? 1 : 0; }
int vb_gemm_gp_tiled_ok(int32_t M, int32_t N) { return vb::gemm_gp_tiled_ok(M, N) ? 1 : 0; }
int vb_gemm(const vb_gemm_args* args, void* stream) {
    if (!args) { vb::set_error("vb_gemm: null args"); return 2; }
    return vb::gemm(*args, static_cast<cudaStream_t>(stream));
}
}
```

visualbert_b200/csrc/vb_internal.h:

```cpp
#pragma once
#include "../../include/vbert_b200.h"
#include "vb_common.cuh"

namespace vb {

int gemm(const vb_gemm_args& a, cudaStream_t st);
bool gemm_gp_tiled_ok(int M, int N);
bool gemm_delta_ok(int M, int N);
int ln_fwd(const void* x, long long ldx, const float* gamma, const float* beta, void* y, long long ldy, float* mean,
           float* rstd, int rows, int H, float eps, cudaStream_t st);
int ln_bwd(const void* dy, const void* x, const float* mean, const float* rstd, const float* gamma, void* dx,
           void* dx_drop, float* dgamma, float* dbeta, float* dbias, int rows, int H, float dropout_p,
           unsigned long long seed, unsigned stream_id, float in_dropout_p, unsigned in_stream_id, cudaStream_t st);
int attn_fwd(const void* qkv, const float* mask_bias, void* ctx, float* lse, void* keep, int B, int S, int A, int H,
             float dropout_p, unsigned long long seed, unsigned stream_id, cudaStream_t st, bool mask_ready = false);
int attn_mask_async(void* keep, int B, int S, int A, int H, float dropout_p, unsigned long long seed, unsigned stream_id,
                    cudaEvent_t before_gemm, cudaStream_t main);
int attn_bwd(const void* qkv, const float* mask_bias, const void* ctx, const float* lse, const void* keep,
             const void* dctx, void* dqkv, float* drow, int B, int S, int A, int H, float dropout_p,
             unsigned long long seed, unsigned stream_id, cudaStream_t st, bool delta_ready = false);
bool attn_bwd_takes_delta(const void* qkv, const void* dctx, void* dqkv, int B, int S, int A, int H);
long long attn_keep_bytes(int B, int S, int A);
int colsum(const void* x, long long ld, float* out, int M, int N, cudaStream_t st);
int cast_f32_bf16(const float* src, void* dst, long long n, cudaStream_t st);
int cast_bf16_f32(const void* src, float* dst, long long n, cudaStream_t st);
int mask_bias(const long long* input_mask, const long long* image_mask, float* out, int B, int T, int V, cudaStream_t st);

struct EmbedParams {
    const long long* ids; const long long* tt; const long long* vt;
    const bf16* vis_proj;
    const float* word; const float* pos; const float* type; const float* pos_vis; const float* type_vis;
    const float* gamma; const float* beta;
    bf16* pre; bf16* y; float* mean; float* rstd;
    int B, T, V, H, vocab, max_pos, n_types;
    float eps;
    float drop_scale; unsigned drop_thresh16; unsigned long long drop_seed; unsigned drop_stream;
};
struct EmbedBwdParams {
    const bf16* de;
    const long long* ids; const long long* tt; const long long* vt;
    float* dword; float* dpos; float* dtype; float* dpos_vis; float* dtype_vis;
    bf16* dvis;
    int B, T, V, H, vocab, max_pos, n_types;
};
int embed_fwd(const EmbedParams& p, cudaStream_t st);
int embed_bwd(const EmbedBwdParams& p, cudaStream_t st);


}
```

Before: 3991.

## Make bf16 GEMM persistent with ping-pong consumer warpgroups and separate wgrad kernel

Replaces the one-tile-per-CTA bf16 GEMM with a persistent kernel whose two consumer warpgroups alternate tiles via named barriers. One warpgroup's epilogue runs while the other issues WGMMA on the next tile, and each tile is fixed at 128x128. Weight-gradient (fp32 output) GEMMs move to a separate kernel that keeps the 128/256 tile choice and uses a new split-K heuristic targeting good SM wave fill. The change adds a lot of scheduling complexity, and the tile-native GELU offset math assumes pairs of 128 tiles, which carries correctness and tuning risk.

```diff
diff --git a/include/vbert_b200.h b/include/vbert_b200.h
--- a/include/vbert_b200.h
+++ b/include/vbert_b200.h
@@ -38,6 +38,7 @@
     const void* delta_ctx; float* delta_out; int32_t delta_seq;
 } vb_gemm_args;
 int vb_gemm_delta_ok(int32_t M, int32_t N);
+int vb_gemm_wgrad_splits(int32_t M, int32_t N, int32_t K);
 int vb_gemm_gp_tiled_ok(int32_t M, int32_t N);
 
 int vb_gemm(const vb_gemm_args* args, void* stream);
diff --git a/visualbert_b200/_lib.py b/visualbert_b200/_lib.py
--- a/visualbert_b200/_lib.py
+++ b/visualbert_b200/_lib.py
@@ -66,7 +66,7 @@
 VB_CAST_CHUNK = 8192
 
 EXPORTS = [
-    "vb_abi_version", "vb_last_error", "vb_launch_count", "vb_profile_enable", "vb_profile_read", "vb_gemm", "vb_gemm_gp_tiled_ok", "vb_gemm_delta_ok", "vb_layernorm_fwd", "vb_layernorm_bwd",
+    "vb_abi_version", "vb_last_error", "vb_launch_count", "vb_profile_enable", "vb_profile_read", "vb_gemm", "vb_gemm_gp_tiled_ok", "vb_gemm_delta_ok", "vb_gemm_wgrad_splits", "vb_layernorm_fwd", "vb_layernorm_bwd",
     "vb_attention_keep_bytes", "vb_attention_fwd", "vb_attention_bwd", "vb_mask_bias", "vb_cast_f32_to_bf16", "vb_cast_bf16_to_f32",
     "vb_colsum_bf16", "vb_cross_entropy_fwd", "vb_cross_entropy_bwd", "vb_layer_fwd", "vb_layer_bwd", "vb_embed_fwd", "vb_embed_bwd",
     "vb_bert_adam_step", "vb_cast_multi", "vb_encoder_arena_layout", "vb_encoder_fwd", "vb_encoder_bwd",
diff --git a/visualbert_b200/csrc/vb_api.cu b/visualbert_b200/csrc/vb_api.cu
--- a/visualbert_b200/csrc/vb_api.cu
+++ b/visualbert_b200/csrc/vb_api.cu
@@ -32,9 +32,7 @@
     memset(&a, 0, sizeof(a));
     a.A = dY; a.lda = N; a.a_mn_major = 1; a.B = X; a.ldb = K; a.b_mn_major = 1;
     a.M = N; a.N = K; a.K = M; a.D = dW; a.ldd = K; a.d_fp32 = 1;
-    const int tiles = ((N + 127) / 128) * ((K + 255) / 256);
-    int splits = (2 * num_sms()) / tiles;
-    a.splits = splits < 1 ? 1 : splits;
+    a.splits = gemm_wgrad_splits(N, K, M);
     return a;
 }
 
diff --git a/visualbert_b200/csrc/vb_common.cuh b/visualbert_b200/csrc/vb_common.cuh
--- a/visualbert_b200/csrc/vb_common.cuh
+++ b/visualbert_b200/csrc/vb_common.cuh
@@ -192,12 +192,17 @@
         : "memory");
     return ok != 0;
 }
+__device__ __forceinline__ uint64_t global_ns() {
+    uint64_t t;
+    asm volatile("mov.u64 %0, %%globaltimer;" : "=l"(t));
+    return t;
+}
 __device__ __forceinline__ void mbar_wait(uint32_t bar, uint32_t parity) {
     if (mbar_try_wait(bar, parity)) return;
-    const long long t0 = clock64();
+    const uint64_t t0 = global_ns();
     uint32_t spins = 0;
     while (!mbar_try_wait(bar, parity)) {
-        if ((++spins & 0x3ffu) == 0 && clock64() - t0 > 4000000000ll) __trap();
+        if ((++spins & 0x3ffu) == 0 && global_ns() - t0 > 10000000000ull) __trap();
     }
 }
 
@@ -291,6 +296,9 @@
 __device__ __forceinline__ void named_bar_sync(int id, int nthreads) {
     asm volatile("bar.sync %0, %1;" ::"r"(id), "r"(nthreads) : "memory");
 }
+__device__ __forceinline__ void named_bar_arrive(int id, int nthreads) {
+    asm volatile("bar.arrive %0, %1;" ::"r"(id), "r"(nthreads) : "memory");
+}
 
 __device__ __forceinline__ uint4 ldg_v4(const void* p) {
     return __ldg(reinterpret_cast<const uint4*>(p));
diff --git a/visualbert_b200/csrc/vb_gemm.cu b/visualbert_b200/csrc/vb_gemm.cu
--- a/visualbert_b200/csrc/vb_gemm.cu
+++ b/visualbert_b200/csrc/vb_gemm.cu
@@ -48,26 +48,22 @@
 }
 
 constexpr int BLOCK_M = 128;
+constexpr int BLOCK_N = 128;
 constexpr int BLOCK_K = 64;
 constexpr int WGMMA_K = 16;
 constexpr int kStages = 4;
-constexpr int kEpiWarps = 8;
-constexpr int kThreads = 128 + kEpiWarps * 32;
+constexpr int kThreads = 384;
 constexpr int kAtomBytes = 64 * BLOCK_K * 2;
-
-template <int BLOCK_N>
-struct Cfg {
-    static constexpr int A_BYTES = BLOCK_M * BLOCK_K * 2;
-    static constexpr int B_BYTES = BLOCK_N * BLOCK_K * 2;
-    static constexpr int STAGE_BYTES = A_BYTES + B_BYTES;
-    static constexpr int ACC_LD = BLOCK_N + 4;
-    static constexpr int RING_BYTES = kStages * STAGE_BYTES > BLOCK_M * ACC_LD * 4 ? kStages * STAGE_BYTES : BLOCK_M * ACC_LD * 4;
-    static constexpr int BAR_OFF = RING_BYTES;
-    static constexpr int NUM_BARS = 2 * kStages;
-    static constexpr int BIAS_OFF = BAR_OFF + NUM_BARS * 8;
-    static constexpr int SMEM_BYTES = BIAS_OFF + BLOCK_N * 4 + 1024;
-    static_assert(SMEM_BYTES <= 227 * 1024, "shared memory per block");
-};
+constexpr int kABytes = BLOCK_M * BLOCK_K * 2;
+constexpr int kStageBytes = kABytes + BLOCK_N * BLOCK_K * 2;
+constexpr int kStgLd = BLOCK_N / 2 + 4;
+constexpr int kStgBytes = BLOCK_M * kStgLd * 4;
+constexpr int kStgOff = kStages * kStageBytes;
+constexpr int kBiasOff = kStgOff + 2 * kStgBytes;
+constexpr int kBarOff = kBiasOff + 2 * BLOCK_N * 4;
+constexpr int kSmemBytes = kBarOff + 2 * kStages * 8 + 1024;
+static_assert(kSmemBytes <= 227 * 1024, "shared memory per block");
+constexpr int kBarMmaTurn = 1, kBarEpi = 3;
 
 struct GemmParams {
     int M, N, K;
@@ -196,12 +192,9 @@
     }
 }
 
-template <bool A_MN, bool B_MN, int BLOCK_N, bool OUT_F32, int EPI = EPI_GENERIC>
+template <bool A_MN, bool B_MN, int EPI = EPI_GENERIC>
 __global__ void __launch_bounds__(kThreads, 1)
 gemm_wgmma_kernel(const __grid_constant__ CUtensorMap tmA, const __grid_constant__ CUtensorMap tmB, const GemmParams p) {
-    using C = Cfg<BLOCK_N>;
-    static_assert(BLOCK_N % 128 == 0, "64 x 128 wgmma pieces");
-    static_assert(!(EPI == EPI_GELU_FWD_T || EPI == EPI_DGELU_BWD_T) || BLOCK_N == 256, "tile-native gelu' is defined on 256-wide tiles");
     extern __shared__ uint8_t smem_raw[];
     const uint32_t raw = smem_u32(smem_raw);
     const uint32_t base = (raw + 1023u) & ~1023u;
@@ -210,10 +203,227 @@
     const int warp = threadIdx.x >> 5;
     const int lane = threadIdx.x & 31;
 
-    auto a_tile = [&](int s) { return base + s * C::STAGE_BYTES; };
-    auto b_tile = [&](int s) { return base + s * C::STAGE_BYTES + C::A_BYTES; };
-    auto full_bar = [&](int s) { return base + C::BAR_OFF + 8 * s; };
-    auto empty_bar = [&](int s) { return base + C::BAR_OFF + 8 * (kStages + s); };
+    auto a_tile = [&](int s) { return base + s * kStageBytes; };
+    auto b_tile = [&](int s) { return base + s * kStageBytes + kABytes; };
+    auto full_bar = [&](int s) { return base + kBarOff + 8 * s; };
+    auto empty_bar = [&](int s) { return base + kBarOff + 8 * (kStages + s); };
+
+    if (threadIdx.x == 0) {
+        tma_prefetch_desc(&tmA);
+        tma_prefetch_desc(&tmB);
+        for (int s = 0; s < kStages; ++s) {
+            mbar_init(full_bar(s), 1);
+            mbar_init(empty_bar(s), 1);
+        }
+        fence_barrier_init();
+    }
+    __syncthreads();
+    pdl_trigger();
+    pdl_wait();
+
+    auto unit_count = [&] { return ((p.M + BLOCK_M - 1) / BLOCK_M) * ((p.N + BLOCK_N - 1) / BLOCK_N) * p.splits; };
+    auto unit = [&](int t) {
+        return decode_tile(t, (p.N + BLOCK_N - 1) / BLOCK_N, p.splits, (p.K + BLOCK_K - 1) / BLOCK_K, (p.M + BLOCK_M - 1) / BLOCK_M, p.m_fast != 0);
+    };
+
+    if (warp < 4) {
+        reg_dec<40>();
+        if (warp == 0) {
+            const int units = unit_count();
+            uint32_t it = 0;
+            for (int t = blockIdx.x; t < units; t += gridDim.x) {
+                const TileCoord tc = unit(t);
+                for (int kb = tc.kb_begin; kb < tc.kb_end; ++kb, ++it) {
+                    const int stage = it % kStages;
+                    mbar_wait(empty_bar(stage), ((it / kStages) & 1u) ^ 1u);
+                    if (elect_one()) {
+                        mbar_arrive_expect_tx(full_bar(stage), kStageBytes);
+                        if constexpr (!A_MN) {
+                            tma_load_2d(a_tile(stage), &tmA, full_bar(stage), kb * BLOCK_K, tc.m_blk * BLOCK_M);
+                        } else {
+#pragma unroll
+                            for (int i = 0; i < BLOCK_M / 64; ++i)
+                                tma_load_2d(a_tile(stage) + i * kAtomBytes, &tmA, full_bar(stage), tc.m_blk * BLOCK_M + i * 64, kb * BLOCK_K);
+                        }
+                        if constexpr (!B_MN) {
+                            tma_load_2d(b_tile(stage), &tmB, full_bar(stage), kb * BLOCK_K, tc.n_blk * BLOCK_N);
+                        } else {
+#pragma unroll
+                            for (int i = 0; i < BLOCK_N / 64; ++i)
+                                tma_load_2d(b_tile(stage) + i * kAtomBytes, &tmB, full_bar(stage), tc.n_blk * BLOCK_N + i * 64, kb * BLOCK_K);
+                        }
+                    }
+                    __syncwarp();
+                }
+            }
+        }
+        return;
+    }
+    reg_inc<232>();
+
+    const int wg = (warp >> 2) - 1;
+    const int q = warp & 3;
+    const int wt = threadIdx.x & 127;
+    float* sstg = reinterpret_cast<float*>(smem + kStgOff + wg * kStgBytes);
+    float* sbias = reinterpret_cast<float*>(smem + kBiasOff) + wg * BLOCK_N;
+    const bool has_bias = p.bias != nullptr;
+    constexpr uint32_t a_kstep = A_MN ? WGMMA_K * 128 : WGMMA_K * 2;
+    constexpr uint32_t b_kstep = B_MN ? WGMMA_K * 128 : WGMMA_K * 2;
+    constexpr bool kEx = EPI != EPI_BIAS && !epi_is_gelu(EPI);
+    constexpr bool kExPre = kEx && EPI != EPI_GENERIC;
+
+    const int units = unit_count();
+    uint32_t it = 0;
+    int j = 0;
+    for (int t = blockIdx.x; t < units; t += gridDim.x, ++j) {
+        const TileCoord tc = unit(t);
+        const int nk = tc.kb_end - tc.kb_begin;
+        if ((j & 1) != wg) { it += nk; continue; }
+
+        float acc[2][64];
+        if (j > 0) named_bar_sync(kBarMmaTurn + wg, 256);
+        for (int kb = 0; kb < nk; ++kb, ++it) {
+            const int stage = it % kStages;
+            mbar_wait(full_bar(stage), (it / kStages) & 1u);
+            const uint32_t a0 = a_tile(stage), b0 = b_tile(stage);
+            wgmma_fence();
+#pragma unroll
+            for (int k = 0; k < BLOCK_K / WGMMA_K; ++k) {
+                const uint64_t bd = wgmma_desc_sw128(b0 + k * b_kstep, kAtomBytes, 1024);
+#pragma unroll
+                for (int h = 0; h < 2; ++h)
+                    wgmma_m64n128k16<A_MN ? 1 : 0, B_MN ? 1 : 0>(acc[h], wgmma_desc_sw128(a0 + h * 8192 + k * a_kstep, kAtomBytes, 1024), bd,
+                                                                 (kb > 0 || k > 0) ? 1u : 0u);
+            }
+            wgmma_commit();
+            wgmma_wait<1>();
+            if (kb > 0 && wt == 0) mbar_arrive(empty_bar((it - 1) % kStages));
+        }
+        if (t + static_cast<int>(gridDim.x) < units) named_bar_arrive(kBarMmaTurn + (wg ^ 1), 256);
+        wgmma_wait<0>();
+        if (wt == 0) mbar_arrive(empty_bar((it - 1) % kStages));
+
+        const int row = tc.m_blk * BLOCK_M + q * 32 + lane;
+        const int col0 = tc.n_blk * BLOCK_N;
+        const long long gp_tile_off =
+            ((((static_cast<long long>(tc.m_blk >> 1) * (p.N >> 8) + (tc.n_blk >> 1)) * 2 + (tc.m_blk & 1)) * 8 + 4 * (tc.n_blk & 1) + q) * 8) * 512 +
+            lane * 16;
+        const bf16* exb = nullptr;
+        long long ex_step = 16;
+        {
+            constexpr bool kWantAdd = EPI == EPI_RESID || EPI == EPI_DROP_RESID || EPI == EPI_DELTA;
+            if (row < p.M) {
+                if (kWantAdd || (EPI == EPI_GENERIC && p.addend != nullptr)) exb = p.addend + static_cast<long long>(row) * p.ld_add + col0;
+                else if (EPI == EPI_DGELU_BWD || (EPI == EPI_GENERIC && p.epilogue == VB_EPI_DGELU))
+                    exb = p.aux_in + static_cast<long long>(row) * p.ld_aux + col0;
+                else if (EPI == EPI_DGELU_BWD_T) { exb = p.aux_in + gp_tile_off; ex_step = 512; }
+            }
+        }
+        const bool bias_mine = p.splits == 1 || (t % p.splits) == 0;
+        [[maybe_unused]] float hsum = 0.f;
+#pragma unroll
+        for (int hh = 0; hh < 2; ++hh) {
+            uint32_t ex[kExPre ? 4 : 1][8];
+            if constexpr (kExPre) {
+#pragma unroll
+                for (int k = 0; k < 4; ++k)
+                    if (exb != nullptr && col0 + (4 * hh + k) * 16 < p.N) ldg_v8(exb + (4 * hh + k) * ex_step, ex[k]);
+            }
+            named_bar_sync(kBarEpi + wg, 128);
+            if (hh == 0 && has_bias) {
+                const int col = col0 + wt;
+                sbias[wt] = (bias_mine && col < p.N) ? __ldg(p.bias + col) : 0.f;
+            }
+            {
+                const int r0 = 16 * q + (lane >> 2);
+#pragma unroll
+                for (int h = 0; h < 2; ++h)
+#pragma unroll
+                    for (int jj = 0; jj < 8; ++jj)
+#pragma unroll
+                        for (int i = 0; i < 2; ++i)
+                            *reinterpret_cast<float2*>(sstg + (64 * h + r0 + 8 * i) * kStgLd + jj * 8 + 2 * (lane & 3)) =
+                                make_float2(acc[h][4 * (8 * hh + jj) + 2 * i], acc[h][4 * (8 * hh + jj) + 2 * i + 1]);
+            }
+            named_bar_sync(kBarEpi + wg, 128);
+
+            const float* srow = sstg + (q * 32 + lane) * kStgLd;
+#pragma unroll
+            for (int kk = 0; kk < 4; ++kk) {
+                const int k = 4 * hh + kk;
+                const int col = col0 + k * 16;
+                if (row < p.M && col < p.N) {
+                    float x[16];
+#pragma unroll
+                    for (int i = 0; i < 4; ++i) {
+                        const float4 v = *reinterpret_cast<const float4*>(srow + kk * 16 + 4 * i);
+                        x[4 * i] = v.x; x[4 * i + 1] = v.y; x[4 * i + 2] = v.z; x[4 * i + 3] = v.w;
+                    }
+                    const float* sb = has_bias ? sbias + k * 16 : nullptr;
+                    if constexpr (kEx && !kExPre) {
+                        if (exb != nullptr) ldg_v8(exb + k * ex_step, ex[0]);
+                    }
+                    const uint32_t (&e)[8] = ex[kExPre ? kk : 0];
+                    if constexpr (EPI == EPI_GELU_FWD_T) {
+                        uint32_t o0[8], o1[8];
+                        epilogue16<false, EPI, true>(p, row, col, sb, e, x, o0, o1);
+                        stg_v8(reinterpret_cast<bf16*>(p.D) + gp_tile_off + k * 512, o0);
+                        stg_v8(p.aux_out + static_cast<long long>(row) * p.ld_aux + col, o1);
+                    } else if constexpr (EPI == EPI_DELTA) {
+                        uint32_t o0[8];
+                        epilogue16<false, EPI, true>(p, row, col, sb, e, x, o0);
+                        stg_v8(reinterpret_cast<bf16*>(p.D) + static_cast<long long>(row) * p.ldd + col, o0);
+#pragma unroll
+                        for (int i = 0; i < 8; ++i) {
+                            const float2 a = unpack_bf16x2(o0[i]), b = unpack_bf16x2(e[i]);
+                            hsum = fmaf(a.x, b.x, fmaf(a.y, b.y, hsum));
+                        }
+                    } else {
+                        epilogue16<false, EPI>(p, row, col, sb, e, x);
+                    }
+                }
+                if constexpr (EPI == EPI_DELTA) {
+                    if (kk == 3) {
+                        const int c4 = col - 48;
+                        if (row < p.M && c4 < p.N) {
+                            const int bi = row / p.delta_seq, si = row - bi * p.delta_seq;
+                            p.delta_out[(static_cast<long long>(bi) * (p.N >> 6) + (c4 >> 6)) * p.delta_seq + si] = hsum;
+                        }
+                        hsum = 0.f;
+                    }
+                }
+            }
+        }
+    }
+}
+
+
+template <int BN>
+struct WgradCfg {
+    static constexpr int STAGE_BYTES = kABytes + BN * BLOCK_K * 2;
+    static constexpr int RING_BYTES = kStages * STAGE_BYTES > BLOCK_M * (BN + 4) * 4 ? kStages * STAGE_BYTES : BLOCK_M * (BN + 4) * 4;
+    static constexpr int SMEM_BYTES = RING_BYTES + 2 * kStages * 8 + BN * 4 + 1024;
+    static_assert(SMEM_BYTES <= 227 * 1024, "shared memory per block");
+};
+
+template <bool A_MN, bool B_MN, int BN>
+__global__ void __launch_bounds__(kThreads, 1)
+gemm_wgrad_kernel(const __grid_constant__ CUtensorMap tmA, const __grid_constant__ CUtensorMap tmB, const GemmParams p) {
+    constexpr int kStage = WgradCfg<BN>::STAGE_BYTES;
+    constexpr int kBar = WgradCfg<BN>::RING_BYTES;
+    constexpr int kBias = kBar + 2 * kStages * 8;
+    constexpr int kAccLd = BN + 4;
+    extern __shared__ uint8_t smem_raw[];
+    const uint32_t raw = smem_u32(smem_raw);
+    const uint32_t base = (raw + 1023u) & ~1023u;
+    uint8_t* smem = smem_raw + (base - raw);
+
+    const int warp = threadIdx.x >> 5;
+    const int lane = threadIdx.x & 31;
+    auto a_tile = [&](int s) { return base + s * kStage; };
+    auto b_tile = [&](int s) { return base + s * kStage + kABytes; };
+    auto full_bar = [&](int s) { return base + kBar + 8 * s; };
+    auto empty_bar = [&](int s) { return base + kBar + 8 * (kStages + s); };
 
     if (threadIdx.x == 0) {
         tma_prefetch_desc(&tmA);
@@ -229,7 +439,7 @@
     pdl_wait();
 
     const int m_blocks = (p.M + BLOCK_M - 1) / BLOCK_M;
-    const int n_blocks = (p.N + BLOCK_N - 1) / BLOCK_N;
+    const int n_blocks = (p.N + BN - 1) / BN;
     const int k_blocks = (p.K + BLOCK_K - 1) / BLOCK_K;
     const TileCoord tc = decode_tile(blockIdx.x, n_blocks, p.splits, k_blocks, m_blocks, p.m_fast != 0);
 
@@ -241,7 +451,7 @@
             for (int kb = tc.kb_begin; kb < tc.kb_end; ++kb) {
                 mbar_wait(empty_bar(stage), phase ^ 1u);
                 if (elect_one()) {
-                    mbar_arrive_expect_tx(full_bar(stage), C::STAGE_BYTES);
+                    mbar_arrive_expect_tx(full_bar(stage), kStage);
                     if constexpr (!A_MN) {
                         tma_load_2d(a_tile(stage), &tmA, full_bar(stage), kb * BLOCK_K, tc.m_blk * BLOCK_M);
                     } else {
@@ -250,11 +460,11 @@
                             tma_load_2d(a_tile(stage) + i * kAtomBytes, &tmA, full_bar(stage), tc.m_blk * BLOCK_M + i * 64, kb * BLOCK_K);
                     }
                     if constexpr (!B_MN) {
-                        tma_load_2d(b_tile(stage), &tmB, full_bar(stage), kb * BLOCK_K, tc.n_blk * BLOCK_N);
+                        tma_load_2d(b_tile(stage), &tmB, full_bar(stage), kb * BLOCK_K, tc.n_blk * BN);
                     } else {
 #pragma unroll
-                        for (int i = 0; i < BLOCK_N / 64; ++i)
-                            tma_load_2d(b_tile(stage) + i * kAtomBytes, &tmB, full_bar(stage), tc.n_blk * BLOCK_N + i * 64, kb * BLOCK_K);
+                        for (int i = 0; i < BN / 64; ++i)
+                            tma_load_2d(b_tile(stage) + i * kAtomBytes, &tmB, full_bar(stage), tc.n_blk * BN + i * 64, kb * BLOCK_K);
                     }
                 }
                 __syncwarp();
@@ -267,16 +477,16 @@
 
     const int wg = (warp >> 2) - 1;
     const int et = threadIdx.x - 128;
-    float* sbias = reinterpret_cast<float*>(smem + C::BIAS_OFF);
+    float* sbias = reinterpret_cast<float*>(smem + kBias);
     const bool has_bias = p.bias != nullptr;
     if (has_bias) {
         const bool mine = p.splits == 1 || (blockIdx.x % p.splits) == 0;
-        for (int i = et; i < BLOCK_N; i += kEpiWarps * 32) {
-            const int col = tc.n_blk * BLOCK_N + i;
+        for (int i = et; i < BN; i += 256) {
+            const int col = tc.n_blk * BN + i;
             sbias[i] = (mine && col < p.N) ? __ldg(p.bias + col) : 0.f;
         }
     }
-    constexpr int NH = BLOCK_N / 128;
+    constexpr int NH = BN / 128;
     constexpr uint32_t a_kstep = A_MN ? WGMMA_K * 128 : WGMMA_K * 2;
     constexpr uint32_t b_kstep = B_MN ? WGMMA_K * 128 : WGMMA_K * 2;
     float acc[NH][64];
@@ -305,33 +515,10 @@
     }
 
     const int ew = warp - 4;
-    const int q = ew & 3, half = ew >> 2;
-    const int lrow = q * 32 + lane;
+    const int lrow = (ew & 3) * 32 + lane, half = ew >> 2;
     const int row = tc.m_blk * BLOCK_M + lrow;
-    const int col0 = tc.n_blk * BLOCK_N + half * (BLOCK_N / 2);
-    constexpr int NCH = BLOCK_N / 2 / 16;
-    const long long gp_tile_off =
-        ((((static_cast<long long>(tc.m_blk >> 1) * n_blocks + tc.n_blk) * 2 + (tc.m_blk & 1)) * kEpiWarps + ew) * NCH) * 512 + lane * 16;
-    const bf16* exb = nullptr;
-    long long ex_step = 16;
-    if constexpr (!OUT_F32) {
-        constexpr bool kWantAdd = EPI == EPI_RESID || EPI == EPI_DROP_RESID || EPI == EPI_DELTA;
-        if (row < p.M) {
-            if (kWantAdd || (EPI == EPI_GENERIC && p.addend != nullptr)) exb = p.addend + static_cast<long long>(row) * p.ld_add + col0;
-            else if (EPI == EPI_DGELU_BWD || (EPI == EPI_GENERIC && p.epilogue == VB_EPI_DGELU))
-                exb = p.aux_in + static_cast<long long>(row) * p.ld_aux + col0;
-            else if (EPI == EPI_DGELU_BWD_T) { exb = p.aux_in + gp_tile_off; ex_step = 512; }
-        }
-    }
-    constexpr bool kEx = !OUT_F32 && EPI != EPI_BIAS && !epi_is_gelu(EPI);
-    uint32_t ex[kEx ? NCH : 1][8];
-    if constexpr (kEx) {
-#pragma unroll
-        for (int k = 0; k < NCH; ++k)
-            if (exb != nullptr && col0 + k * 16 < p.N) ldg_v8(exb + k * ex_step, ex[k]);
-    }
-
-    named_bar_sync(1, kEpiWarps * 32);
+    const int col0 = tc.n_blk * BN + half * (BN / 2);
+    named_bar_sync(1, 256);
     float* sacc = reinterpret_cast<float*>(smem);
     {
         const int r0 = wg * 64 + ((warp & 3) << 4) + (lane >> 2);
@@ -341,15 +528,14 @@
             for (int j = 0; j < 16; ++j)
 #pragma unroll
                 for (int i = 0; i < 2; ++i)
-                    *reinterpret_cast<float2*>(sacc + (r0 + 8 * i) * C::ACC_LD + h * 128 + j * 8 + 2 * (lane & 3)) =
+                    *reinterpret_cast<float2*>(sacc + (r0 + 8 * i) * kAccLd + h * 128 + j * 8 + 2 * (lane & 3)) =
                         make_float2(acc[h][4 * j + 2 * i], acc[h][4 * j + 2 * i + 1]);
     }
-    named_bar_sync(1, kEpiWarps * 32);
-
-    const float* srow = sacc + lrow * C::ACC_LD + half * (BLOCK_N / 2);
-    [[maybe_unused]] float hsum = 0.f;
-#pragma unroll
-    for (int k = 0; k < NCH; ++k) {
+    named_bar_sync(1, 256);
+    const float* srow = sacc + lrow * kAccLd + half * (BN / 2);
+    const uint32_t none[8] = {0, 0, 0, 0, 0, 0, 0, 0};
+#pragma unroll
+    for (int k = 0; k < BN / 2 / 16; ++k) {
         const int col = col0 + k * 16;
         if (row < p.M && col < p.N) {
             float x[16];
@@ -358,35 +544,7 @@
                 const float4 v = *reinterpret_cast<const float4*>(srow + k * 16 + 4 * i);
                 x[4 * i] = v.x; x[4 * i + 1] = v.y; x[4 * i + 2] = v.z; x[4 * i + 3] = v.w;
             }
-            const float* sb = has_bias ? sbias + half * (BLOCK_N / 2) + k * 16 : nullptr;
-            const uint32_t (&e)[8] = ex[kEx ? k : 0];
-            if constexpr (EPI == EPI_GELU_FWD_T) {
-                uint32_t o0[8], o1[8];
-                epilogue16<OUT_F32, EPI, true>(p, row, col, sb, e, x, o0, o1);
-                stg_v8(reinterpret_cast<bf16*>(p.D) + gp_tile_off + k * 512, o0);
-                stg_v8(p.aux_out + static_cast<long long>(row) * p.ld_aux + col, o1);
-            } else if constexpr (EPI == EPI_DELTA) {
-                uint32_t o0[8];
-                epilogue16<OUT_F32, EPI, true>(p, row, col, sb, e, x, o0);
-                stg_v8(reinterpret_cast<bf16*>(p.D) + static_cast<long long>(row) * p.ldd + col, o0);
-#pragma unroll
-                for (int i = 0; i < 8; ++i) {
-                    const float2 a = unpack_bf16x2(o0[i]), b = unpack_bf16x2(e[i]);
-                    hsum = fmaf(a.x, b.x, fmaf(a.y, b.y, hsum));
-                }
-            } else {
-                epilogue16<OUT_F32, EPI>(p, row, col, sb, e, x);
-            }
-        }
-        if constexpr (EPI == EPI_DELTA) {
-            if ((k & 3) == 3) {
-                const int c4 = col - 48;
-                if (row < p.M && c4 < p.N) {
-                    const int bi = row / p.delta_seq, si = row - bi * p.delta_seq;
-                    p.delta_out[(static_cast<long long>(bi) * (p.N >> 6) + (c4 >> 6)) * p.delta_seq + si] = hsum;
-                }
-                hsum = 0.f;
-            }
+            epilogue16<true>(p, row, col, has_bias ? sbias + half * (BN / 2) + k * 16 : nullptr, none, x);
         }
     }
 }
@@ -474,20 +632,53 @@
     return n[dev];
 }
 
-template <bool A_MN, bool B_MN, int BLOCK_N, bool OUT_F32, int EPI = EPI_GENERIC>
+template <bool A_MN, bool B_MN, int EPI = EPI_GENERIC>
 static int launch(const CUtensorMap& ta, const CUtensorMap& tb, const GemmParams& p, cudaStream_t st) {
-    using C = Cfg<BLOCK_N>;
-    auto kern = gemm_wgmma_kernel<A_MN, B_MN, BLOCK_N, OUT_F32, EPI>;
+    auto kern = gemm_wgmma_kernel<A_MN, B_MN, EPI>;
     static int configured[kMaxDevices] = {0};
-    VB_CHECK_CUDA(ensure_dyn_smem(kern, C::SMEM_BYTES, configured));
-    const long long tiles = static_cast<long long>((p.M + BLOCK_M - 1) / BLOCK_M) * ((p.N + BLOCK_N - 1) / BLOCK_N) * p.splits;
+    VB_CHECK_CUDA(ensure_dyn_smem(kern, kSmemBytes, configured));
+    const long long units = static_cast<long long>((p.M + BLOCK_M - 1) / BLOCK_M) * ((p.N + BLOCK_N - 1) / BLOCK_N);
+    VB_REQUIRE(units < (1LL << 31), "vb_gemm: too many tiles");
+    const int grid = units < num_sms() ? static_cast<int>(units) : num_sms();
+    {
+        ProfScope ps(st, B_MN ? PROF_GEMM_DGRAD : PROF_GEMM_FWD, 2.0 * p.M * p.N * p.K, 1);
+        VB_CHECK_CUDA(launch_pdl(kern, dim3(static_cast<unsigned>(grid)), dim3(kThreads), kSmemBytes, st, ta, tb, p));
+    }
+    VB_CHECK_CUDA(cudaGetLastError());
+    return 0;
+}
+
+static int wgrad_block_n(int N) { return (N >= 256 && ((N + 255) / 256 * 256 - N) * 8 <= N) ? 256 : 128; }
+
+template <bool A_MN, bool B_MN, int BN>
+static int launch_wgrad(const CUtensorMap& ta, const CUtensorMap& tb, const GemmParams& p, cudaStream_t st) {
+    auto kern = gemm_wgrad_kernel<A_MN, B_MN, BN>;
+    static int configured[kMaxDevices] = {0};
+    VB_CHECK_CUDA(ensure_dyn_smem(kern, WgradCfg<BN>::SMEM_BYTES, configured));
+    const long long tiles = static_cast<long long>((p.M + BLOCK_M - 1) / BLOCK_M) * ((p.N + BN - 1) / BN) * p.splits;
     VB_REQUIRE(tiles < (1LL << 31), "vb_gemm: too many tiles");
     {
-        ProfScope ps(st, OUT_F32 ? PROF_GEMM_WGRAD : (B_MN ? PROF_GEMM_DGRAD : PROF_GEMM_FWD), 2.0 * p.M * p.N * p.K, 1);
-        VB_CHECK_CUDA(launch_pdl(kern, dim3(static_cast<unsigned>(tiles)), dim3(kThreads), C::SMEM_BYTES, st, ta, tb, p));
+        ProfScope ps(st, PROF_GEMM_WGRAD, 2.0 * p.M * p.N * p.K, 1);
+        VB_CHECK_CUDA(launch_pdl(kern, dim3(static_cast<unsigned>(tiles)), dim3(kThreads), WgradCfg<BN>::SMEM_BYTES, st, ta, tb, p));
     }
     VB_CHECK_CUDA(cudaGetLastError());
     return 0;
+}
+
+int gemm_wgrad_splits(int M, int N, int K) {
+    const long long tiles = static_cast<long long>((M + BLOCK_M - 1) / BLOCK_M) * ((N + wgrad_block_n(N) - 1) / wgrad_block_n(N));
+    const int k_blocks = (K + BLOCK_K - 1) / BLOCK_K;
+    const long long sms = num_sms();
+    const int max_splits = k_blocks / 8 > 1 ? k_blocks / 8 : 1;
+    int best = 1;
+    double best_fill = 0.0;
+    for (int s = 1; s <= max_splits; ++s) {
+        const long long ctas = tiles * s, slots = (ctas + sms - 1) / sms * sms;
+        const double fill = static_cast<double>(ctas) / static_cast<double>(slots);
+        if (fill >= 0.8) return s;
+        if (fill > best_fill) { best_fill = fill; best = s; }
+    }
+    return best;
 }
 
 bool pdl_enabled() {
@@ -554,7 +745,8 @@
     }
     {
         static const int order_off = [] { const char* e = getenv("VB_GEMM_TILE_ORDER"); return (e != nullptr && atoi(e) == 0) ? 1 : 0; }();
-        p.m_fast = (!order_off && (a.M + BLOCK_M - 1) / BLOCK_M < (a.N + 255) / 256) ? 1 : 0;
+        const int bn = a.d_fp32 ? wgrad_block_n(a.N) : BLOCK_N;
+        p.m_fast = (!order_off && (a.M + BLOCK_M - 1) / BLOCK_M < (a.N + bn - 1) / bn) ? 1 : 0;
     }
     if (a.dropout_p > 0.0f) {
         const DropQ q = dropout_quantise(a.dropout_p);
@@ -564,20 +756,16 @@
         p.drop_stream = a.dropout_stream;
     }
 
-    const int n_pad256 = (a.N + 255) / 256 * 256;
-    const bool bn256 = (a.N >= 256) && ((n_pad256 - a.N) * 8 <= a.N);
-    VB_REQUIRE(!a.delta_out || bn256, "vb_gemm: delta_out needs 256-wide tiles");
-
     CUtensorMap ta, tb;
     int rc;
     if (!a.a_mn_major) rc = make_tmap_bf16(&ta, a.A, a.K, a.M, a.lda, BLOCK_M);
     else               rc = make_tmap_bf16(&ta, a.A, a.M, a.K, a.lda, BLOCK_K);
     if (rc) return rc;
-    if (!a.b_mn_major) rc = make_tmap_bf16(&tb, a.B, a.K, a.N, a.ldb, bn256 ? 256 : 128);
+    if (!a.b_mn_major) rc = make_tmap_bf16(&tb, a.B, a.K, a.N, a.ldb, a.d_fp32 ? wgrad_block_n(a.N) : BLOCK_N);
     else               rc = make_tmap_bf16(&tb, a.B, a.N, a.K, a.ldb, BLOCK_K);
     if (rc) return rc;
 
-    if (bn256 && !a.d_fp32) {
+    if (!a.d_fp32) {
         const bool drop = a.dropout_p > 0.0f, add = a.addend != nullptr;
         int epi = EPI_GENERIC;
         if (a.epilogue == VB_EPI_GELU && !drop && !add) epi = a.gp_tiled ? EPI_GELU_FWD_T : EPI_GELU_FWD;
@@ -588,40 +776,34 @@
                    "vb_gemm: gp_tiled needs a plain GELU / DGELU epilogue (no dropout, no addend)");
         if (!a.a_mn_major && !a.b_mn_major) {
             switch (epi) {
-                case EPI_BIAS: return launch<false, false, 256, false, EPI_BIAS>(ta, tb, p, st);
-                case EPI_RESID: return launch<false, false, 256, false, EPI_RESID>(ta, tb, p, st);
-                case EPI_DROP_RESID: return launch<false, false, 256, false, EPI_DROP_RESID>(ta, tb, p, st);
-                case EPI_GELU_FWD: return launch<false, false, 256, false, EPI_GELU_FWD>(ta, tb, p, st);
-                case EPI_GELU_FWD_T: return launch<false, false, 256, false, EPI_GELU_FWD_T>(ta, tb, p, st);
-                default: return launch<false, false, 256, false>(ta, tb, p, st);
+                case EPI_BIAS: return launch<false, false, EPI_BIAS>(ta, tb, p, st);
+                case EPI_RESID: return launch<false, false, EPI_RESID>(ta, tb, p, st);
+                case EPI_DROP_RESID: return launch<false, false, EPI_DROP_RESID>(ta, tb, p, st);
+                case EPI_GELU_FWD: return launch<false, false, EPI_GELU_FWD>(ta, tb, p, st);
+                case EPI_GELU_FWD_T: return launch<false, false, EPI_GELU_FWD_T>(ta, tb, p, st);
+                default: return launch<false, false>(ta, tb, p, st);
             }
         }
         if (!a.a_mn_major && a.b_mn_major) {
             switch (epi) {
-                case EPI_BIAS: return launch<false, true, 256, false, EPI_BIAS>(ta, tb, p, st);
-                case EPI_RESID: return launch<false, true, 256, false, EPI_RESID>(ta, tb, p, st);
-                case EPI_DGELU_BWD: return launch<false, true, 256, false, EPI_DGELU_BWD>(ta, tb, p, st);
-                case EPI_DELTA: return launch<false, true, 256, false, EPI_DELTA>(ta, tb, p, st);
-                case EPI_DGELU_BWD_T: return launch<false, true, 256, false, EPI_DGELU_BWD_T>(ta, tb, p, st);
-                default: return launch<false, true, 256, false>(ta, tb, p, st);
-            }
-        }
-    }
-
-#define VB_DISPATCH(AM, BM, F32)                                         \
-    (bn256 ? launch<AM, BM, 256, F32>(ta, tb, p, st) : launch<AM, BM, 128, F32>(ta, tb, p, st))
-    if (!a.d_fp32) {
-        if (!a.a_mn_major && !a.b_mn_major) return VB_DISPATCH(false, false, false);
-        if (!a.a_mn_major && a.b_mn_major) return VB_DISPATCH(false, true, false);
-        if (a.a_mn_major && a.b_mn_major) return VB_DISPATCH(true, true, false);
-        return VB_DISPATCH(true, false, false);
-    } else {
-        if (!a.a_mn_major && !a.b_mn_major) return VB_DISPATCH(false, false, true);
-        if (!a.a_mn_major && a.b_mn_major) return VB_DISPATCH(false, true, true);
-        if (a.a_mn_major && a.b_mn_major) return VB_DISPATCH(true, true, true);
-        return VB_DISPATCH(true, false, true);
-    }
-#undef VB_DISPATCH
+                case EPI_BIAS: return launch<false, true, EPI_BIAS>(ta, tb, p, st);
+                case EPI_RESID: return launch<false, true, EPI_RESID>(ta, tb, p, st);
+                case EPI_DGELU_BWD: return launch<false, true, EPI_DGELU_BWD>(ta, tb, p, st);
+                case EPI_DELTA: return launch<false, true, EPI_DELTA>(ta, tb, p, st);
+                case EPI_DGELU_BWD_T: return launch<false, true, EPI_DGELU_BWD_T>(ta, tb, p, st);
+                default: return launch<false, true>(ta, tb, p, st);
+            }
+        }
+        if (a.a_mn_major && a.b_mn_major) return launch<true, true>(ta, tb, p, st);
+        return launch<true, false>(ta, tb, p, st);
+    }
+#define VB_WGRAD(AM, BM) \
+    (wgrad_block_n(a.N) == 256 ? launch_wgrad<AM, BM, 256>(ta, tb, p, st) : launch_wgrad<AM, BM, 128>(ta, tb, p, st))
+    if (!a.a_mn_major && !a.b_mn_major) return VB_WGRAD(false, false);
+    if (!a.a_mn_major && a.b_mn_major) return VB_WGRAD(false, true);
+    if (a.a_mn_major && a.b_mn_major) return VB_WGRAD(true, true);
+    return VB_WGRAD(true, false);
+#undef VB_WGRAD
 }
 
 }
@@ -649,6 +831,7 @@
 }
 int vb_gemm_delta_ok(int32_t M, int32_t N) { return vb::gemm_delta_ok(M, N) ? 1 : 0; }
 int vb_gemm_gp_tiled_ok(int32_t M, int32_t N) { return vb::gemm_gp_tiled_ok(M, N) ? 1 : 0; }
+int vb_gemm_wgrad_splits(int32_t M, int32_t N, int32_t K) { return vb::gemm_wgrad_splits(M, N, K); }
 int vb_gemm(const vb_gemm_args* args, void* stream) {
     if (!args) { vb::set_error("vb_gemm: null args"); return 2; }
     return vb::gemm(*args, static_cast<cudaStream_t>(stream));
diff --git a/visualbert_b200/csrc/vb_internal.h b/visualbert_b200/csrc/vb_internal.h
--- a/visualbert_b200/csrc/vb_internal.h
+++ b/visualbert_b200/csrc/vb_internal.h
@@ -7,6 +7,7 @@
 int gemm(const vb_gemm_args& a, cudaStream_t st);
 bool gemm_gp_tiled_ok(int M, int N);
 bool gemm_delta_ok(int M, int N);
+int gemm_wgrad_splits(int M, int N, int K);
 int ln_fwd(const void* x, long long ldx, const float* gamma, const float* beta, void* y, long long ldy, float* mean,
            float* rstd, int rows, int H, float eps, cudaStream_t st);
 int ln_bwd(const void* dy, const void* x, const float* mean, const float* rstd, const float* gamma, void* dx,
```

New measurement: 4059, median of 6. +1.7%, better.
